# yzhang511/multi_modal_foundation_model

Hardware: NVIDIA B200
Metric: train trials/sec fwd+bwd (higher is better)
Workload: dtype bf16

## Files before the change

include/mmfm_b200.h:

```cpp
#ifndef MMFM_B200_H_
#define MMFM_B200_H_

#include <stddef.h>
#include <stdint.h>

#ifdef __cplusplus
extern "C" {
#endif

#define MMFM_ABI_VERSION 5

const char* mmfm_last_error(void);
int mmfm_abi_version(void);
int mmfm_sm_count(void);

typedef struct mmfm_dropout {
  const unsigned long long* seed;
  uint32_t site;
  uint32_t thresh;
  float scale;
} mmfm_dropout;

enum mmfm_act {
  MMFM_ACT_NONE = 0,
  MMFM_ACT_GELU = 1,
  MMFM_ACT_SOFTSIGN = 2,
  MMFM_ACT_DGELU = 3,
  MMFM_ACT_DSOFTSIGN = 4,
  MMFM_ACT_GELU_DG = 5,
  MMFM_ACT_MULAUX = 6,
  MMFM_ACT_ROWDOT_DROP = 7
};

typedef struct mmfm_gemm_args {
  const void* A; long long lda;
  const void* B; long long ldb;
  int M, N, K;
  void* D; long long ldd;
  int d_fp32;
  void* D2;
  const float* bias;
  const float* res; long long ldr;
  const void* aux; long long ldaux;
  int act; float act_scale;
  mmfm_dropout drop;
  int remap_T, remap_S, remap_off;
  const unsigned char* row_zero;
  float* rowdot; int rowdot_S;
} mmfm_gemm_args;

int mmfm_gemm_tn(const mmfm_gemm_args* args, void* stream);

int mmfm_gemm_wgrad(const void* dY, long long lddy, const void* X, long long ldx, int R, int NO, int KI, float* dW,
                    long long ldw, float* dbias, void* stream);
int mmfm_colsum_bf16(const void* dY, long long ld, int R, int NO, float* out, void* stream);

int mmfm_cast_bf16(const float* x, long long ldx, void* y, long long ldy, void* yt, long long ldyt, int R, int C,
                   void* stream);

int mmfm_layernorm_fwd(const float* x, const float* gamma, const float* beta, void* y, float* mean, float* rstd,
                       int R, int H, float eps, int modmajor_T, int S, void* stream);
int mmfm_layernorm_bwd(const void* dy, const float* x, const float* mean, const float* rstd, const float* gamma,
                       const float* dres, float* dx, void* dxb, const mmfm_dropout* drop, float* dgamma,
                       float* dbeta, int R, int H, int modmajor_T, int S, void* stream);

#define MMFM_MAX_LN 8
typedef struct {
  const float* x;
  int R, H, n;
  float eps;
  const float* gamma[MMFM_MAX_LN];
  const float* beta[MMFM_MAX_LN];
  void* y[MMFM_MAX_LN];
  float* mean;
  float* rstd;
  const void* dy[MMFM_MAX_LN];
  float* dgamma[MMFM_MAX_LN];
  float* dbeta[MMFM_MAX_LN];
  float* dx;
  void* dxb;
} mmfm_ln_multi_args;
int mmfm_layernorm_fwd_multi(const mmfm_ln_multi_args* a, void* stream);
int mmfm_layernorm_bwd_multi(const mmfm_ln_multi_args* a, void* stream);

int mmfm_scalenorm_fwd(const float* x, const float* g, void* y, float* rnorm, int R, int H, float eps, void* stream);
int mmfm_scalenorm_bwd(const void* dy, const float* x, const float* rnorm, const float* g, const float* dres, float* dx,
                       void* dxb, const mmfm_dropout* drop, float* dg, int R, int H, float eps, void* stream);

enum mmfm_mask_mode {
  MMFM_MASK_KEY = 0,
  MMFM_MASK_KEY_OR_DIAG = 1,
  MMFM_MASK_CAUSAL = 2
};
typedef struct mmfm_attn_args {
  const void* q; long long ldq;
  const void* k; long long ldk;
  const void* v; long long ldv;
  void* o; long long ldo;
  float* lse;
  const unsigned char* key_valid;
  const short* mod_q; const short* mod_k;
  int B, n_heads, Sq, Sk, d_head;
  int mask_mode;
  float scale;
  mmfm_dropout drop_p;
  mmfm_dropout drop_o;
  unsigned short* p_keep;
  void* d_o; long long lddo;
  float* delta;
  void* dq; long long lddq;
  void* dk; long long lddk;
  void* dv; long long lddv;
  int prep_done;
} mmfm_attn_args;
int mmfm_attention_fwd(const mmfm_attn_args* args, void* stream);
int mmfm_attention_bwd(const mmfm_attn_args* args, void* stream);

#define MMFM_MAX_MOD 8
typedef struct mmfm_mask_args {
  int n_mod, B, T;
  const long long* mask[MMFM_MAX_MOD]; long long mask_sb[MMFM_MAX_MOD]; long long mask_st[MMFM_MAX_MOD];
  const long long* attn[MMFM_MAX_MOD]; long long attn_sb[MMFM_MAX_MOD]; long long attn_st[MMFM_MAX_MOD];
  int channels[MMFM_MAX_MOD];
  const unsigned int* sample_thresh;
  const unsigned long long* seed;
} mmfm_mask_args;
#define MMFM_MASK_SITE 8192u
int mmfm_mask_prep(const mmfm_mask_args* args, unsigned char* zero_flags, unsigned char* key_valid,
                   unsigned char* tok_mask, long long* n_examples, float* inv_n, void* stream);
int mmfm_embed_assemble(const float* mod_emb_row, const float* pos_embed, const long long* ts, float* emb, int B,
                        int T, int S, int off, int H, void* stream);
int mmfm_embed_assemble_bwd(const float* g, const float* g2, const long long* ts, float* dpos, float* dmod, int B,
                            int T, int S, int off, int H, void* stream);
int mmfm_embed_grad_prep(const float* dx, void* dtok, const unsigned char* row_zero, const mmfm_dropout* drop, int B,
                         int T, int S, int off, int H, void* stream);
int mmfm_smallc_embed_fwd(const float* in, const float* W1, const float* b1, const float* W2, const float* b2,
                          const float* emb, float* x, float* hid, const unsigned char* row_zero,
                          const mmfm_dropout* drop, float act_scale, int act, int B, int T, int S, int off, int C,
                          int H, void* stream);
int mmfm_smallc_embed_bwd(const float* in, const float* hid, const float* W2, const float* dx,
                          const unsigned char* row_zero, const mmfm_dropout* drop, float act_scale, int act,
                          float* dW1, float* db1, float* dW2, float* db2, int B, int T, int S, int off, int C, int H,
                          void* stream);
int mmfm_smallc_head_fwd(const void* y, const float* W, const float* b, float* preds, int R, int H, int C,
                         void* stream);
int mmfm_smallc_head_bwd(const void* y, const float* W, const void* dpreds, long long lddp, void* dy, float* dW,
                         float* db, int R, int H, int C, void* stream);

enum mmfm_loss_kind {
  MMFM_LOSS_POISSON = 0, MMFM_LOSS_MSE = 1,
  MMFM_LOSS_CE = 2
};
int mmfm_loss_fwd_bwd(const float* preds, const float* targets, const unsigned char* tok_mask, int S, int off,
                      const float* inv_n, int kind, int B, int T, int C, float* partials, int n_partials, void* dpreds,
                      long long lddp, void* stream);
int mmfm_loss_finalize(const float* partials, int n_partials, int n_mod, const float* inv_n, float* mod_loss,
                       float* loss, void* stream);

typedef struct mmfm_cast_item {
  const float* src; long long ld_src;
  void* dst; long long ld_dst;
  void* dst_t; long long ld_dst_t;
  int rows, cols;
  int tile_start;
  int pad_;
} mmfm_cast_item;
int mmfm_cast_bf16_multi(const mmfm_cast_item* items_dev, int n_items, int total_tiles, void* stream);
int mmfm_scale_inplace(float* x, long long n, const float* scale_dev, void* stream);

int mmfm_csr_to_dense_u8(const unsigned char* data, const int* indices, const long long* row_ptr, long long n_rows, int N,
                         unsigned char* out, void* stream);
int mmfm_u8_expand(const unsigned char* x, long long R, int C, float* y32, long long ld32, void* y16, long long ld16,
                   void* stream);

int mmfm_column_stats(const float* pred, const float* y, long long R, int C, int log_rate, double* out, void* stream);

int mmfm_adamw_step(float* p, const float* g, float* exp_avg, float* exp_avg_sq, long long n, float lr, float beta1,
                    float beta2, float eps, float weight_decay, long long step, void* stream);

typedef struct mmfm_det_ws {
  void* buf;
  long long bytes;
  unsigned int* tickets;
  int n_tickets;
} mmfm_det_ws;
enum mmfm_det_kind {
  MMFM_DET_WGRAD = 0,
  MMFM_DET_COLSUM = 1,
  MMFM_DET_LN_BWD = 2,
  MMFM_DET_LN_BWD_MULTI = 3,
  MMFM_DET_SCALENORM_BWD = 4,
  MMFM_DET_EMBED_ASM_BWD = 5,
  MMFM_DET_SMALLC_EMBED_BWD = 6,
  MMFM_DET_SMALLC_HEAD_BWD = 7,
  MMFM_DET_COLUMN_STATS = 8
};
int mmfm_det_ws_bytes(int kind, long long d0, long long d1, long long d2, long long* bytes, int* n_tickets);
int mmfm_gemm_wgrad_det(const void* dY, long long lddy, const void* X, long long ldx, int R, int NO, int KI, float* dW,
                        long long ldw, float* dbias, const mmfm_det_ws* ws, void* stream);
int mmfm_colsum_bf16_det(const void* dY, long long ld, int R, int NO, float* out, const mmfm_det_ws* ws, void* stream);
int mmfm_layernorm_bwd_det(const void* dy, const float* x, const float* mean, const float* rstd, const float* gamma,
                           const float* dres, float* dx, void* dxb, const mmfm_dropout* drop, float* dgamma,
                           float* dbeta, int R, int H, int modmajor_T, int S, const mmfm_det_ws* ws, void* stream);
int mmfm_layernorm_bwd_multi_det(const mmfm_ln_multi_args* a, const mmfm_det_ws* ws, void* stream);
// ... 19 lines not shown
```

multi_modal_foundation_model_b200/_lib.py:

```python
from __future__ import annotations

import ctypes as C
import os
import subprocess
import sys
from typing import List, Optional

_PKG_DIR = os.path.dirname(os.path.abspath(__file__))
_CSRC = os.path.join(_PKG_DIR, "csrc")
LIB_PATH = os.environ.get("MMFM_LIB_PATH") or os.path.join(_PKG_DIR, "libmmfm_b200.so")
SOURCES = ["host_util.cu", "gemm.cu", "gemm_ts.cu", "norm.cu", "attention.cu", "attention_pipe.cu", "attention_bwd_stream.cu", "attention_bwd_persist.cu", "attention_bwd_ws.cu", "glue.cu"]
NVCC_FLAGS = ["-gencode", "arch=compute_100a,code=sm_100a", "-lineinfo", "-O3", "-std=c++17", "-Xcompiler", "-fPIC",
              "-Xptxas", "-v"]

MAX_MOD = 8
ABI_VERSION = 5
MASK_SITE = 8192


def _nvcc() -> str:
    for p in (os.environ.get("NVCC"), "/usr/local/cuda/bin/nvcc", "nvcc"):
        if p and (os.path.isabs(p) and os.path.exists(p) or not os.path.isabs(p)):
            return p
    return "nvcc"


def needs_build() -> bool:
    if not os.path.exists(LIB_PATH):
        return True
    t = os.path.getmtime(LIB_PATH)
    deps = [os.path.join(_CSRC, f) for f in os.listdir(_CSRC)]
    deps.append(os.path.join(os.path.dirname(_PKG_DIR), "include", "mmfm_b200.h"))
    return any(os.path.getmtime(d) > t for d in deps if os.path.exists(d))


def build(force: bool = False, verbose: bool = False) -> str:
    if not force and not needs_build():
        return LIB_PATH
    objs: List[str] = []
    build_dir = os.path.join(_PKG_DIR, "build")
    os.makedirs(build_dir, exist_ok=True)
    procs = []
    for src in SOURCES:
        obj = os.path.join(build_dir, src.replace(".cu", ".o"))
        objs.append(obj)
        extra = os.environ.get("MMFM_NVCC_EXTRA", "").split()
        cmd = [_nvcc(), *NVCC_FLAGS, *extra, "-c", os.path.join(_CSRC, src), "-o", obj]
        procs.append((src, subprocess.Popen(cmd, stdout=subprocess.PIPE, stderr=subprocess.STDOUT, text=True)))
    for src, p in procs:
        out, _ = p.communicate()
        if verbose or p.returncode != 0:
            sys.stderr.write(out)
        if p.returncode != 0:
            raise RuntimeError(f"nvcc failed on {src}")
    cmd = [_nvcc(), "-shared", "-o", LIB_PATH, *objs, "-lcudart"]
    r = subprocess.run(cmd, stdout=subprocess.PIPE, stderr=subprocess.STDOUT, text=True)
    if r.returncode != 0:
        sys.stderr.write(r.stdout)
        raise RuntimeError("link of libmmfm_b200.so failed")
    return LIB_PATH


class Dropout(C.Structure):
    _fields_ = [("seed", C.c_void_p), ("site", C.c_uint32), ("thresh", C.c_uint32), ("scale", C.c_float)]


class GemmArgs(C.Structure):
    _fields_ = [
        ("A", C.c_void_p), ("lda", C.c_longlong),
        ("B", C.c_void_p), ("ldb", C.c_longlong),
        ("M", C.c_int), ("N", C.c_int), ("K", C.c_int),
        ("D", C.c_void_p), ("ldd", C.c_longlong),
        ("d_fp32", C.c_int),
        ("D2", C.c_void_p),
        ("bias", C.c_void_p),
        ("res", C.c_void_p), ("ldr", C.c_longlong),
        ("aux", C.c_void_p), ("ldaux", C.c_longlong),
        ("act", C.c_int), ("act_scale", C.c_float),
        ("drop", Dropout),
        ("remap_T", C.c_int), ("remap_S", C.c_int), ("remap_off", C.c_int),
        ("row_zero", C.c_void_p),
        ("rowdot", C.c_void_p), ("rowdot_S", C.c_int),
    ]


class AttnArgs(C.Structure):
    _fields_ = [
        ("q", C.c_void_p), ("ldq", C.c_longlong),
        ("k", C.c_void_p), ("ldk", C.c_longlong),
        ("v", C.c_void_p), ("ldv", C.c_longlong),
        ("o", C.c_void_p), ("ldo", C.c_longlong),
        ("lse", C.c_void_p),
        ("key_valid", C.c_void_p),
        ("mod_q", C.c_void_p), ("mod_k", C.c_void_p),
        ("B", C.c_int), ("n_heads", C.c_int), ("Sq", C.c_int), ("Sk", C.c_int), ("d_head", C.c_int),
        ("mask_mode", C.c_int),
        ("scale", C.c_float),
        ("drop_p", Dropout), ("drop_o", Dropout),
        ("p_keep", C.c_void_p),
        ("d_o", C.c_void_p), ("lddo", C.c_longlong),
        ("delta", C.c_void_p),
        ("dq", C.c_void_p), ("lddq", C.c_longlong),
        ("dk", C.c_void_p), ("lddk", C.c_longlong),
        ("dv", C.c_void_p), ("lddv", C.c_longlong),
        ("prep_done", C.c_int),
    ]


class MaskArgs(C.Structure):
    _fields_ = [
        ("n_mod", C.c_int), ("B", C.c_int), ("T", C.c_int),
        ("mask", C.c_void_p * MAX_MOD), ("mask_sb", C.c_longlong * MAX_MOD), ("mask_st", C.c_longlong * MAX_MOD),
        ("attn", C.c_void_p * MAX_MOD), ("attn_sb", C.c_longlong * MAX_MOD), ("attn_st", C.c_longlong * MAX_MOD),
        ("channels", C.c_int * MAX_MOD),
        ("sample_thresh", C.c_void_p), ("seed", C.c_void_p),
    ]


MAX_LN = 8


class LnMultiArgs(C.Structure):
    _fields_ = [
        ("x", C.c_void_p), ("R", C.c_int), ("H", C.c_int), ("n", C.c_int), ("eps", C.c_float),
        ("gamma", C.c_void_p * MAX_LN), ("beta", C.c_void_p * MAX_LN), ("y", C.c_void_p * MAX_LN),
        ("mean", C.c_void_p), ("rstd", C.c_void_p),
        ("dy", C.c_void_p * MAX_LN), ("dgamma", C.c_void_p * MAX_LN), ("dbeta", C.c_void_p * MAX_LN),
        ("dx", C.c_void_p), ("dxb", C.c_void_p),
    ]


class CastItem(C.Structure):
    _fields_ = [
        ("src", C.c_void_p), ("ld_src", C.c_longlong),
        ("dst", C.c_void_p), ("ld_dst", C.c_longlong),
        ("dst_t", C.c_void_p), ("ld_dst_t", C.c_longlong),
        ("rows", C.c_int), ("cols", C.c_int),
        ("tile_start", C.c_int), ("pad_", C.c_int),
    ]


class DetWs(C.Structure):
    _fields_ = [("buf", C.c_void_p), ("bytes", C.c_longlong), ("tickets", C.c_void_p), ("n_tickets", C.c_int)]


ACT_NONE, ACT_GELU, ACT_SOFTSIGN, ACT_DGELU, ACT_DSOFTSIGN, ACT_GELU_DG, ACT_MULAUX, ACT_ROWDOT_DROP = 0, 1, 2, 3, 4, 5, 6, 7
MASK_KEY, MASK_KEY_OR_DIAG, MASK_CAUSAL = 0, 1, 2
LOSS_POISSON, LOSS_MSE, LOSS_CE = 0, 1, 2
(DET_WGRAD, DET_COLSUM, DET_LN_BWD, DET_LN_BWD_MULTI, DET_SCALENORM_BWD, DET_EMBED_ASM_BWD, DET_SMALLC_EMBED_BWD,
 DET_SMALLC_HEAD_BWD, DET_COLUMN_STATS) = range(9)

_vp, _i, _ll, _f = C.c_void_p, C.c_int, C.c_longlong, C.c_float
_DP = C.POINTER(Dropout)
_WS = C.POINTER(DetWs)

SIGNATURES = {
    "mmfm_gemm_tn": [C.POINTER(GemmArgs), _vp],
    "mmfm_gemm_wgrad": [_vp, _ll, _vp, _ll, _i, _i, _i, _vp, _ll, _vp, _vp],
    "mmfm_colsum_bf16": [_vp, _ll, _i, _i, _vp, _vp],
    "mmfm_cast_bf16": [_vp, _ll, _vp, _ll, _vp, _ll, _i, _i, _vp],
    "mmfm_cast_bf16_multi": [_vp, _i, _i, _vp],
    "mmfm_scale_inplace": [_vp, _ll, _vp, _vp],
    "mmfm_csr_to_dense_u8": [_vp, _vp, _vp, _ll, _i, _vp, _vp],
    "mmfm_u8_expand": [_vp, _ll, _i, _vp, _ll, _vp, _ll, _vp],
    "mmfm_column_stats": [_vp, _vp, _ll, _i, _i, _vp, _vp],
    "mmfm_adamw_step": [_vp, _vp, _vp, _vp, _ll, _f, _f, _f, _f, _f, _ll, _vp],
    "mmfm_layernorm_fwd": [_vp, _vp, _vp, _vp, _vp, _vp, _i, _i, _f, _i, _i, _vp],
    "mmfm_layernorm_bwd": [_vp, _vp, _vp, _vp, _vp, _vp, _vp, _vp, _DP, _vp, _vp, _i, _i, _i, _i, _vp],
    "mmfm_layernorm_fwd_multi": [C.POINTER(LnMultiArgs), _vp],
    "mmfm_layernorm_bwd_multi": [C.POINTER(LnMultiArgs), _vp],
    "mmfm_scalenorm_fwd": [_vp, _vp, _vp, _vp, _i, _i, _f, _vp],
    "mmfm_scalenorm_bwd": [_vp, _vp, _vp, _vp, _vp, _vp, _vp, _DP, _vp, _i, _i, _f, _vp],
    "mmfm_attention_fwd": [C.POINTER(AttnArgs), _vp],
    "mmfm_attention_bwd": [C.POINTER(AttnArgs), _vp],
    "mmfm_mask_prep": [C.POINTER(MaskArgs), _vp, _vp, _vp, _vp, _vp, _vp],
    "mmfm_embed_assemble": [_vp, _vp, _vp, _vp, _i, _i, _i, _i, _i, _vp],
    "mmfm_embed_assemble_bwd": [_vp, _vp, _vp, _vp, _vp, _i, _i, _i, _i, _i, _vp],
    "mmfm_embed_grad_prep": [_vp, _vp, _vp, _DP, _i, _i, _i, _i, _i, _vp],
    "mmfm_smallc_embed_fwd": [_vp, _vp, _vp, _vp, _vp, _vp, _vp, _vp, _vp, _DP, _f, _i, _i, _i, _i, _i, _i, _i, _vp],
    "mmfm_smallc_embed_bwd": [_vp, _vp, _vp, _vp, _vp, _DP, _f, _i, _vp, _vp, _vp, _vp, _i, _i, _i, _i, _i, _i, _vp],
    "mmfm_smallc_head_fwd": [_vp, _vp, _vp, _vp, _i, _i, _i, _vp],
    "mmfm_smallc_head_bwd": [_vp, _vp, _vp, _ll, _vp, _vp, _vp, _i, _i, _i, _vp],
    "mmfm_loss_fwd_bwd": [_vp, _vp, _vp, _i, _i, _vp, _i, _i, _i, _i, _vp, _i, _vp, _ll, _vp],
    "mmfm_loss_finalize": [_vp, _i, _i, _vp, _vp, _vp, _vp],
    "mmfm_det_ws_bytes": [_i, _ll, _ll, _ll, C.POINTER(C.c_longlong), C.POINTER(C.c_int)],
    "mmfm_gemm_wgrad_det": [_vp, _ll, _vp, _ll, _i, _i, _i, _vp, _ll, _vp, _WS, _vp],
    "mmfm_colsum_bf16_det": [_vp, _ll, _i, _i, _vp, _WS, _vp],
    "mmfm_layernorm_bwd_det": [_vp, _vp, _vp, _vp, _vp, _vp, _vp, _vp, _DP, _vp, _vp, _i, _i, _i, _i, _WS, _vp],
    "mmfm_layernorm_bwd_multi_det": [C.POINTER(LnMultiArgs), _WS, _vp],
    "mmfm_scalenorm_bwd_det": [_vp, _vp, _vp, _vp, _vp, _vp, _vp, _DP, _vp, _i, _i, _f, _WS, _vp],
    "mmfm_embed_assemble_bwd_det": [_vp, _vp, _vp, _vp, _vp, _i, _i, _i, _i, _i, _i, _WS, _vp],
    "mmfm_smallc_embed_bwd_det": [_vp, _vp, _vp, _vp, _vp, _DP, _f, _i, _vp, _vp, _vp, _vp, _i, _i, _i, _i, _i, _i, _WS,
                                  _vp],
    "mmfm_smallc_head_bwd_det": [_vp, _vp, _vp, _ll, _vp, _vp, _vp, _i, _i, _i, _WS, _vp],
    "mmfm_column_stats_det": [_vp, _vp, _ll, _i, _i, _vp, _WS, _vp],
}
_SPECIAL = {
    "mmfm_last_error": ([], C.c_char_p),
    "mmfm_abi_version": ([], C.c_int),
    "mmfm_sm_count": ([], C.c_int),
}
EXPORTED_SYMBOLS = sorted(list(SIGNATURES) + list(_SPECIAL))

_LIB: Optional[C.CDLL] = None


class MmfmError(RuntimeError):
    pass


def lib() -> C.CDLL:
    global _LIB
    if _LIB is not None:
        return _LIB
    if not os.path.exists(LIB_PATH):
        raise MmfmError(
            f"{LIB_PATH} is missing: build it with `python -c 'import __graft_entry__ as g; g.build()'` "
            "(nvcc, sm_100a).  The B200 path has no CPU / PyTorch fallback.")
    L = C.CDLL(LIB_PATH)
    for name, argtypes in SIGNATURES.items():
        fn = getattr(L, name)
        fn.argtypes = argtypes
        fn.restype = C.c_int
    for name, (argtypes, restype) in _SPECIAL.items():
        fn = getattr(L, name)
        fn.argtypes = argtypes
        fn.restype = restype
    if L.mmfm_abi_version() != ABI_VERSION:
        raise MmfmError("libmmfm_b200.so ABI version mismatch")
    _LIB = L
    return L


def check(rc: int, what: str = "") -> None:
    if rc != 0:
        msg = lib().mmfm_last_error()
        raise MmfmError(f"{what} failed (rc={rc}): {msg.decode() if msg else '?'}")
```

multi_modal_foundation_model_b200/csrc/common.cuh:

```cuda
#pragma once
#include <cuda.h>
#include <cuda_bf16.h>
#include <cuda_runtime.h>
#include <stdint.h>
#include <stdio.h>

namespace mmfm {

typedef __nv_bfloat16 bf16;

#define MMFM_DEVINL __device__ __forceinline__

MMFM_DEVINL uint32_t smem_u32(const void* p) { return (uint32_t)__cvta_generic_to_shared(p); }

MMFM_DEVINL bool elect_one() {
  uint32_t pred = 0;
  asm volatile(
      "{\n\t.reg .pred P1;\n\t.reg .b32 R1;\n\t"
      "elect.sync R1|P1, 0xffffffff;\n\t"
      "selp.u32 %0, 1, 0, P1;\n\t}\n"
      : "=r"(pred));
  return pred != 0;
}

// ... 161 lines not shown
}

MMFM_DEVINL void tmem_ld32(uint32_t taddr, uint32_t (&r)[32]) {
  asm volatile(
      "tcgen05.ld.sync.aligned.32x32b.x32.b32 "
      "{%0, %1, %2, %3, %4, %5, %6, %7, %8, %9, %10, %11, %12, %13, %14, %15, "
      "%16, %17, %18, %19, %20, %21, %22, %23, %24, %25, %26, %27, %28, %29, %30, %31}, [%32];"
      : "=r"(r[0]), "=r"(r[1]), "=r"(r[2]), "=r"(r[3]), "=r"(r[4]), "=r"(r[5]), "=r"(r[6]), "=r"(r[7]),
        "=r"(r[8]), "=r"(r[9]), "=r"(r[10]), "=r"(r[11]), "=r"(r[12]), "=r"(r[13]), "=r"(r[14]), "=r"(r[15]),
        "=r"(r[16]), "=r"(r[17]), "=r"(r[18]), "=r"(r[19]), "=r"(r[20]), "=r"(r[21]), "=r"(r[22]),
        "=r"(r[23]), "=r"(r[24]), "=r"(r[25]), "=r"(r[26]), "=r"(r[27]), "=r"(r[28]), "=r"(r[29]),
        "=r"(r[30]), "=r"(r[31])
      : "r"(taddr)
      : "memory");
}
MMFM_DEVINL void tmem_ld16(uint32_t taddr, uint32_t (&r)[16]) {
  asm volatile(
      "tcgen05.ld.sync.aligned.32x32b.x16.b32 "
      "{%0, %1, %2, %3, %4, %5, %6, %7, %8, %9, %10, %11, %12, %13, %14, %15}, [%16];"
      : "=r"(r[0]), "=r"(r[1]), "=r"(r[2]), "=r"(r[3]), "=r"(r[4]), "=r"(r[5]), "=r"(r[6]), "=r"(r[7]),
        "=r"(r[8]), "=r"(r[9]), "=r"(r[10]), "=r"(r[11]), "=r"(r[12]), "=r"(r[13]), "=r"(r[14]), "=r"(r[15])
      : "r"(taddr)
      : "memory");
}
MMFM_DEVINL void tmem_ld_wait() { asm volatile("tcgen05.wait::ld.sync.aligned;" ::: "memory"); }
MMFM_DEVINL void tmem_st16(uint32_t taddr, const uint32_t (&r)[16]) {
  asm volatile(
      "tcgen05.st.sync.aligned.32x32b.x16.b32 [%0], "
      "{%1, %2, %3, %4, %5, %6, %7, %8, %9, %10, %11, %12, %13, %14, %15, %16};" ::"r"(taddr),
      "r"(r[0]), "r"(r[1]), "r"(r[2]), "r"(r[3]), "r"(r[4]), "r"(r[5]), "r"(r[6]), "r"(r[7]), "r"(r[8]), "r"(r[9]),
      "r"(r[10]), "r"(r[11]), "r"(r[12]), "r"(r[13]), "r"(r[14]), "r"(r[15])
      : "memory");
}
MMFM_DEVINL void tmem_st8(uint32_t taddr, const uint32_t (&r)[8]) {
  asm volatile("tcgen05.st.sync.aligned.32x32b.x8.b32 [%0], {%1, %2, %3, %4, %5, %6, %7, %8};" ::"r"(taddr), "r"(r[0]),
               "r"(r[1]), "r"(r[2]), "r"(r[3]), "r"(r[4]), "r"(r[5]), "r"(r[6]), "r"(r[7])
               : "memory");
}
MMFM_DEVINL void tmem_st_wait() { asm volatile("tcgen05.wait::st.sync.aligned;" ::: "memory"); }

MMFM_DEVINL uint64_t make_smem_desc(uint32_t saddr, uint32_t lbo_bytes, uint32_t sbo_bytes, uint32_t layout) {
  uint64_t d = 0;
  d |= (uint64_t)((saddr >> 4) & 0x3FFF);
  d |= (uint64_t)((lbo_bytes >> 4) & 0x3FFF) << 16;
  d |= (uint64_t)((sbo_bytes >> 4) & 0x3FFF) << 32;
  d |= (uint64_t)1 << 46;
  d |= (uint64_t)(layout & 7) << 61;
  return d;
}
__host__ __device__ inline uint32_t make_idesc_bf16(uint32_t M, uint32_t N, uint32_t a_mn, uint32_t b_mn) {
  uint32_t d = 0;
  d |= 1u << 4;
  d |= 1u << 7;
  d |= 1u << 10;
  d |= (a_mn & 1u) << 15;
  d |= (b_mn & 1u) << 16;
  d |= ((N >> 3) & 0x3F) << 17;
  d |= ((M >> 4) & 0x1F) << 24;
  return d;
}

constexpr int kPhiloxRounds = 7;

MMFM_DEVINL void mulhilo32(uint32_t a, uint32_t b, uint32_t& hi, uint32_t& lo) {
  const unsigned long long p = (unsigned long long)a * (unsigned long long)b;
  hi = (uint32_t)(p >> 32);
  lo = (uint32_t)p;
}

MMFM_DEVINL uint4 philox4x32(uint32_t c0, uint32_t c1, uint32_t c2, uint32_t c3, uint32_t k0, uint32_t k1) {
#pragma unroll
  for (int r = 0; r < kPhiloxRounds; ++r) {
    uint32_t hi0, lo0, hi1, lo1;
    mulhilo32(0xD2511F53u, c0, hi0, lo0);
    mulhilo32(0xCD9E8D57u, c2, hi1, lo1);
    const uint32_t n0 = hi1 ^ c1 ^ k0;
    const uint32_t n2 = hi0 ^ c3 ^ k1;
    c0 = n0; c1 = lo1; c2 = n2; c3 = lo0;
    k0 += 0x9E3779B9u; k1 += 0xBB67AE85u;
  }
  return make_uint4(c0, c1, c2, c3);
}

MMFM_DEVINL void philox4x32_x4(uint32_t c0, uint32_t c1, uint32_t c2, uint32_t c3, uint32_t k0, uint32_t k1,
                               uint4 (&out)[4]) {
  uint32_t a0[4], a1[4], a2[4], a3[4];
#pragma unroll
  for (int q = 0; q < 4; ++q) { a0[q] = c0 + q; a1[q] = c1; a2[q] = c2; a3[q] = c3; }
#pragma unroll
  for (int r = 0; r < kPhiloxRounds; ++r) {
#pragma unroll
    for (int q = 0; q < 4; ++q) {
      uint32_t hi0, lo0, hi1, lo1;
      mulhilo32(0xD2511F53u, a0[q], hi0, lo0);
      mulhilo32(0xCD9E8D57u, a2[q], hi1, lo1);
      const uint32_t n0 = hi1 ^ a1[q] ^ k0;
      const uint32_t n2 = hi0 ^ a3[q] ^ k1;
      a0[q] = n0; a1[q] = lo1; a2[q] = n2; a3[q] = lo0;
    }
    k0 += 0x9E3779B9u; k1 += 0xBB67AE85u;
  }
#pragma unroll
  for (int q = 0; q < 4; ++q) out[q] = make_uint4(a0[q], a1[q], a2[q], a3[q]);
}

struct DropCfg {
  const unsigned long long* seed;
  uint32_t site;
  uint32_t thresh;
  float scale;
};

MMFM_DEVINL uint4 drop_bytes16(unsigned long long seed, uint32_t site, uint64_t row, uint32_t groups_per_row,
                               uint32_t g16) {
  uint64_t g = row * (uint64_t)groups_per_row + g16;
  return philox4x32((uint32_t)g, (uint32_t)(g >> 32), site, 0u, (uint32_t)seed, (uint32_t)(seed >> 32));
}
MMFM_DEVINL uint32_t drop_byte(const uint4& w, int b) {
  uint32_t word = (b < 4) ? w.x : (b < 8) ? w.y : (b < 12) ? w.z : w.w;
  return (word >> ((b & 3) * 8)) & 0xFFu;
}

MMFM_DEVINL float erf_poly(float z, float& e) {
  const float az = fabsf(z);
  float t, ex;
  asm("rcp.approx.ftz.f32 %0, %1;" : "=f"(t) : "f"(fmaf(0.3275911f, az, 1.0f)));
  asm("ex2.approx.ftz.f32 %0, %1;" : "=f"(ex) : "f"(-1.4426950408889634f * z * z));
  e = ex;
  const float poly =
      fmaf(fmaf(fmaf(fmaf(1.061405429f, t, -1.453152027f), t, 1.421413741f), t, -0.284496736f), t, 0.254829592f) * t;
  return copysignf(fmaf(-poly, ex, 1.0f), z);
}
MMFM_DEVINL float gelu_erf(float x) {
  float e;
  return 0.5f * x * (1.0f + erf_poly(x * 0.70710678118654752f, e));
}
MMFM_DEVINL float gelu_erf_grad(float x) {
  float e;
  const float cdf = 0.5f * (1.0f + erf_poly(x * 0.70710678118654752f, e));
  return fmaf(x * 0.3989422804014327f, e, cdf);
}
MMFM_DEVINL void gelu_erf_both(float x, float& g, float& dg) {
  float e;
  const float cdf = 0.5f * (1.0f + erf_poly(x * 0.70710678118654752f, e));
  g = x * cdf;
  dg = fmaf(x * 0.3989422804014327f, e, cdf);
}
MMFM_DEVINL float softsign(float x) { return x / (1.0f + fabsf(x)); }

MMFM_DEVINL float warp_sum(float v) {
#pragma unroll
  for (int o = 16; o > 0; o >>= 1) v += __shfl_xor_sync(0xffffffffu, v, o);
  return v;
}

MMFM_DEVINL uint32_t pack_bf16x2(float lo, float hi) {
  __nv_bfloat162 v = __floats2bfloat162_rn(lo, hi);
  return *reinterpret_cast<uint32_t*>(&v);
}
MMFM_DEVINL float2 unpack_bf16x2(uint32_t u) {
  __nv_bfloat162 v = *reinterpret_cast<__nv_bfloat162*>(&u);
  return __bfloat1622float2(v);
}


MMFM_DEVINL uint64_t pack_f2(float lo, float hi) {
  uint64_t r;
  asm("mov.b64 %0, {%1, %2};" : "=l"(r) : "f"(lo), "f"(hi));
  return r;
}
MMFM_DEVINL void unpack_f2(uint64_t v, float& lo, float& hi) { asm("mov.b64 {%0, %1}, %2;" : "=f"(lo), "=f"(hi) : "l"(v)); }
MMFM_DEVINL uint64_t ffma2(uint64_t a, uint64_t b, uint64_t c) {
  uint64_t d;
  asm("fma.rn.f32x2 %0, %1, %2, %3;" : "=l"(d) : "l"(a), "l"(b), "l"(c));
  return d;
}
MMFM_DEVINL uint64_t fmul2(uint64_t a, uint64_t b) {
  uint64_t d;
  asm("mul.rn.f32x2 %0, %1, %2;" : "=l"(d) : "l"(a), "l"(b));
  return d;
}
MMFM_DEVINL uint64_t fadd2(uint64_t a, uint64_t b) {
  uint64_t d;
  asm("add.rn.f32x2 %0, %1, %2;" : "=l"(d) : "l"(a), "l"(b));
  return d;
}

MMFM_DEVINL void gelu_erf_both2(float x0, float x1, float& g0, float& g1, float& d0, float& d1) {
  const uint64_t x = pack_f2(x0, x1);
  const uint64_t z = fmul2(x, pack_f2(0.70710678118654752f, 0.70710678118654752f));
  float z0, z1;
  unpack_f2(z, z0, z1);
  float t0, t1, e0, e1;
  asm("rcp.approx.ftz.f32 %0, %1;" : "=f"(t0) : "f"(fmaf(0.3275911f, fabsf(z0), 1.0f)));
  asm("rcp.approx.ftz.f32 %0, %1;" : "=f"(t1) : "f"(fmaf(0.3275911f, fabsf(z1), 1.0f)));
  float a0, a1;
  unpack_f2(fmul2(fmul2(z, z), pack_f2(-1.4426950408889634f, -1.4426950408889634f)), a0, a1);
  asm("ex2.approx.ftz.f32 %0, %1;" : "=f"(e0) : "f"(a0));
  asm("ex2.approx.ftz.f32 %0, %1;" : "=f"(e1) : "f"(a1));
  const uint64_t t = pack_f2(t0, t1), e = pack_f2(e0, e1);
  uint64_t q = ffma2(pack_f2(1.061405429f, 1.061405429f), t, pack_f2(-1.453152027f, -1.453152027f));
  q = ffma2(q, t, pack_f2(1.421413741f, 1.421413741f));
  q = ffma2(q, t, pack_f2(-0.284496736f, -0.284496736f));
  q = ffma2(q, t, pack_f2(0.254829592f, 0.254829592f));
  q = fmul2(q, t);
  float r0, r1;
  unpack_f2(ffma2(q, fmul2(e, pack_f2(-1.0f, -1.0f)), pack_f2(1.0f, 1.0f)), r0, r1);
  const uint64_t erf2 = pack_f2(copysignf(r0, z0), copysignf(r1, z1));
  const uint64_t cdf = ffma2(erf2, pack_f2(0.5f, 0.5f), pack_f2(0.5f, 0.5f));
  unpack_f2(fmul2(x, cdf), g0, g1);
  unpack_f2(ffma2(fmul2(x, pack_f2(0.3989422804014327f, 0.3989422804014327f)), e, cdf), d0, d1);
}

MMFM_DEVINL void ldsm_x4(uint32_t (&r)[4], uint32_t saddr) {
  asm volatile("ldmatrix.sync.aligned.m8n8.x4.shared.b16 {%0,%1,%2,%3}, [%4];"
               : "=r"(r[0]), "=r"(r[1]), "=r"(r[2]), "=r"(r[3])
               : "r"(saddr));
}
MMFM_DEVINL void ldsm_x4_t(uint32_t (&r)[4], uint32_t saddr) {
  asm volatile("ldmatrix.sync.aligned.m8n8.x4.trans.shared.b16 {%0,%1,%2,%3}, [%4];"
               : "=r"(r[0]), "=r"(r[1]), "=r"(r[2]), "=r"(r[3])
               : "r"(saddr));
}
MMFM_DEVINL void mma_16816(float (&d)[4], const uint32_t (&a)[4], const uint32_t (&b)[2]) {
  asm volatile(
      "mma.sync.aligned.m16n8k16.row.col.f32.bf16.bf16.f32 {%0,%1,%2,%3}, {%4,%5,%6,%7}, {%8,%9}, {%0,%1,%2,%3};"
      : "+f"(d[0]), "+f"(d[1]), "+f"(d[2]), "+f"(d[3])
      : "r"(a[0]), "r"(a[1]), "r"(a[2]), "r"(a[3]), "r"(b[0]), "r"(b[1]));
}

MMFM_DEVINL void mma_16816_z(float (&d)[4], const uint32_t (&a)[4], const uint32_t (&b)[2]) {
  asm volatile(
      "mma.sync.aligned.m16n8k16.row.col.f32.bf16.bf16.f32 {%0,%1,%2,%3}, {%4,%5,%6,%7}, {%8,%9}, {%10,%10,%10,%10};"
      : "=f"(d[0]), "=f"(d[1]), "=f"(d[2]), "=f"(d[3])
      : "r"(a[0]), "r"(a[1]), "r"(a[2]), "r"(a[3]), "r"(b[0]), "r"(b[1]), "f"(0.f));
}

MMFM_DEVINL float quad_sum(float v) {
  v += __shfl_xor_sync(0xffffffffu, v, 1);
  v += __shfl_xor_sync(0xffffffffu, v, 2);
  return v;
}
MMFM_DEVINL float quad_max(float v) {
  v = fmaxf(v, __shfl_xor_sync(0xffffffffu, v, 1));
  v = fmaxf(v, __shfl_xor_sync(0xffffffffu, v, 2));
  return v;
}

MMFM_DEVINL float det_add(float a, float b) { return a + b; }
MMFM_DEVINL double det_add(double a, double b) { return a + b; }
MMFM_DEVINL float4 det_add(float4 a, float4 b) { return make_float4(a.x + b.x, a.y + b.y, a.z + b.z, a.w + b.w); }

template <typename V, typename Emit>
MMFM_DEVINL void det_tree_fold(V* ws, long long stride, int n, int leaf, int n_leaves, unsigned int* tickets,
                               Emit emit) {
  __shared__ unsigned int s_second;
  int node = leaf;
  for (int l = 0; (1 << l) < n_leaves; ++l) {
    const int width = (n_leaves + (1 << l) - 1) >> l;
    if ((node | 1) >= width) { node >>= 1; continue; }
    const int right = (node | 1) << l;
    __syncthreads();
    if (threadIdx.x == 0) {
      __threadfence();
      const unsigned int t = atomicAdd(tickets + right - 1, 1u);
      if (t != 0u) {
        tickets[right - 1] = 0u;
        __threadfence();
      }
      s_second = t;
    }
    __syncthreads();
    if (s_second == 0u) return;
    V* a = ws + (long long)((node & ~1) << l) * stride;
    const V* b = ws + (long long)right * stride;
    constexpr int kU = 8;
    for (int i0 = threadIdx.x; i0 < n; i0 += kU * blockDim.x) {
      V va[kU], vb[kU];
#pragma unroll
      for (int u = 0; u < kU; ++u) {
        const int i = i0 + u * blockDim.x;
        if (i < n) { va[u] = __ldcg(a + i); vb[u] = __ldcg(b + i); }
      }
#pragma unroll
      for (int u = 0; u < kU; ++u) {
        const int i = i0 + u * blockDim.x;
        if (i >= n) break;
        if (width == 2) emit(i, det_add(va[u], vb[u]));
        else a[i] = det_add(va[u], vb[u]);
      }
    }
    if (width == 2) return;
    node >>= 1;
  }
  __syncthreads();
  for (int i = threadIdx.x; i < n; i += blockDim.x) emit(i, __ldcg(ws + (long long)leaf * stride + i));
}

MMFM_DEVINL uint32_t drop_byte_at(unsigned long long seed, uint32_t site, uint64_t row, uint32_t groups_per_row,
                                  uint32_t col) {
  uint4 w = drop_bytes16(seed, site, row, groups_per_row, col >> 4);
  return drop_byte(w, col & 15);
}

}
```

multi_modal_foundation_model_b200/csrc/gemm.cu:

```cuda
#include "common.cuh"
#include <stdlib.h>
#include "host_util.h"
#include "../../include/mmfm_b200.h"

namespace mmfm {

constexpr int kBM = 128;
constexpr int kBK = 64;
constexpr int kGemmThreads = 192;

MMFM_DEVINL float4 ld4_f32(const float* p, bool vec, int nvalid) {
  if (vec) return __ldg(reinterpret_cast<const float4*>(p));
  float4 r = make_float4(0.f, 0.f, 0.f, 0.f);
  if (nvalid > 0) r.x = __ldg(p);
  if (nvalid > 1) r.y = __ldg(p + 1);
  if (nvalid > 2) r.z = __ldg(p + 2);
  if (nvalid > 3) r.w = __ldg(p + 3);
  return r;
}
MMFM_DEVINL float4 ld4_bf16(const bf16* p, bool vec, int nvalid) {
  if (vec) {
    const uint2 u = __ldg(reinterpret_cast<const uint2*>(p));
    const float2 a = unpack_bf16x2(u.x), b = unpack_bf16x2(u.y);
    return make_float4(a.x, a.y, b.x, b.y);
  }
  float4 r = make_float4(0.f, 0.f, 0.f, 0.f);
  if (nvalid > 0) r.x = __bfloat162float(p[0]);
  if (nvalid > 1) r.y = __bfloat162float(p[1]);
  if (nvalid > 2) r.z = __bfloat162float(p[2]);
  if (nvalid > 3) r.w = __bfloat162float(p[3]);
  return r;
}
MMFM_DEVINL void st4_f32(float* p, bool vec, int nvalid, const float4& v) {
  if (vec) { *reinterpret_cast<float4*>(p) = v; return; }
  if (nvalid > 0) p[0] = v.x;
  if (nvalid > 1) p[1] = v.y;
  if (nvalid > 2) p[2] = v.z;
  if (nvalid > 3) p[3] = v.w;
}
MMFM_DEVINL void st4_bf16(bf16* p, bool vec, int nvalid, const float4& v) {
  if (vec) { *reinterpret_cast<uint2*>(p) = make_uint2(pack_bf16x2(v.x, v.y), pack_bf16x2(v.z, v.w)); return; }
  if (nvalid > 0) p[0] = __float2bfloat16_rn(v.x);
  if (nvalid > 1) p[1] = __float2bfloat16_rn(v.y);
  if (nvalid > 2) p[2] = __float2bfloat16_rn(v.z);
  if (nvalid > 3) p[3] = __float2bfloat16_rn(v.w);
}

constexpr int kEpiWarps = 16;
constexpr int kTnThreads = 64 + kEpiWarps * 32;

enum EpiKind : int {
  EPI_PLAIN_BF16 = 0,
  EPI_PLAIN_F32 = 1,
  EPI_RES_F32 = 2,
  EPI_GELU = 3,
  EPI_SOFTSIGN = 4,
  EPI_DGELU = 5,
  EPI_DSOFTSIGN = 6,
  EPI_GENERIC = 7,
  EPI_GELU_DG = 8,
  EPI_MULAUX = 9
};

template <int BN, int STAGES, int EPI>
__global__ void __launch_bounds__(kTnThreads, 1) gemm_tn_kernel(const __grid_constant__ CUtensorMap tmA,
                                                                 const __grid_constant__ CUtensorMap tmB,
                                                                 const mmfm_gemm_args p, int tiles_n, int n_tiles,
                                                                 int bstat) {
  constexpr uint32_t kABytes = kBM * kBK * 2;
  constexpr uint32_t kBBytes = BN * kBK * 2;
  constexpr uint32_t kStageBytes = kABytes + kBBytes;
  constexpr uint32_t kTmemCols = 2 * BN;
  constexpr int kPitch = BN + 4;
  constexpr int kHalf = BN / (kEpiWarps / 4);
  constexpr bool GEN = EPI == EPI_GENERIC;

  constexpr int kMaxStages = 8;
  extern __shared__ uint8_t smem_raw[];
  __shared__ __align__(8) uint64_t full_bar[kMaxStages];
  __shared__ __align__(8) uint64_t empty_bar[kMaxStages];
  __shared__ __align__(8) uint64_t b_full;
  __shared__ __align__(8) uint64_t acc_full[2];
  __shared__ __align__(8) uint64_t acc_empty[2];
  __shared__ uint32_t tmem_slot;
  __shared__ __align__(16) float s_bias[kEpiWarps][kHalf];

  const uint32_t smem_base = (smem_u32(smem_raw) + 1023u) & ~1023u;
  float* stage_f = reinterpret_cast<float*>(smem_raw + (smem_base - smem_u32(smem_raw)) + STAGES * kStageBytes);
  const int warp = threadIdx.x >> 5;
  const int lane = threadIdx.x & 31;
  const int nkb = (p.K + kBK - 1) / kBK;
  const uint32_t b_res_bytes = bstat ? (uint32_t)nkb * kBBytes : 0u;
  const uint32_t ring_base = smem_base + b_res_bytes;
  const uint32_t st_bytes = bstat ? kABytes : kStageBytes;
  uint32_t nst = bstat ? (STAGES * kStageBytes - b_res_bytes) / kABytes : (uint32_t)STAGES;
  if (nst > (uint32_t)kMaxStages) nst = kMaxStages;

  pdl_trigger();
  if (warp == 0 && lane == 0) {
    tma_prefetch_desc(&tmA);
    tma_prefetch_desc(&tmB);
#pragma unroll
    for (int s = 0; s < kMaxStages; ++s) {
      mbar_init(&full_bar[s], 1);
      mbar_init(&empty_bar[s], 1);
    }
    mbar_init(&b_full, 1);
    mbar_init(&acc_full[0], 1);
    mbar_init(&acc_full[1], 1);
    mbar_init(&acc_empty[0], kEpiWarps);
    mbar_init(&acc_empty[1], kEpiWarps);
    fence_mbar_init();
  }
  if (warp == 1) {
    tmem_alloc(&tmem_slot, kTmemCols);
    tmem_relinquish();
  }
  tc_fence_before();
  __syncthreads();
  tc_fence_after();
  const uint32_t tmem_base = tmem_slot;
  pdl_wait();

  if (warp == 0) {
    if (elect_one()) {
      uint32_t it = 0;
      if (bstat) {
        const int n0 = ((int)blockIdx.x % tiles_n) * BN;
        mbar_arrive_expect_tx(&b_full, b_res_bytes);
        for (int kb = 0; kb < nkb; ++kb) tma_load_2d_addr(smem_base + kb * kBBytes, &tmB, &b_full, kb * kBK, n0);
      }
      for (int tile = blockIdx.x; tile < n_tiles; tile += gridDim.x) {
        const int m0 = (tile / tiles_n) * kBM, n0 = (tile % tiles_n) * BN;
        {
          const int t2 = tile + 2 * (int)gridDim.x;
          if (t2 < n_tiles && (t2 % tiles_n == 0 || tiles_n > (int)gridDim.x)) {
            const int m2 = (t2 / tiles_n) * kBM;
            for (int kb = 0; kb < nkb; ++kb) tma_prefetch_l2_2d(&tmA, kb * kBK, m2);
          }
        }
        for (int kb = 0; kb < nkb; ++kb, ++it) {
          const uint32_t s = it % nst;
          if (it >= nst) mbar_wait(&empty_bar[s], ((it / nst) - 1) & 1);
          mbar_arrive_expect_tx(&full_bar[s], st_bytes);
          const uint32_t a_dst = ring_base + s * st_bytes;
          tma_load_2d_addr(a_dst, &tmA, &full_bar[s], kb * kBK, m0);
          if (!bstat) tma_load_2d_addr(a_dst + kABytes, &tmB, &full_bar[s], kb * kBK, n0);
        }
      }
    }
  } else if (warp == 1) {
    if (elect_one()) {
      const uint32_t idesc = make_idesc_bf16(kBM, BN, 0, 0);
      uint32_t it = 0, t = 0;
      if (bstat) mbar_wait(&b_full, 0);
      for (int tile = blockIdx.x; tile < n_tiles; tile += gridDim.x, ++t) {
        const uint32_t buf = t & 1u;
        if (t >= 2) mbar_wait(&acc_empty[buf], ((t >> 1) - 1) & 1);
        tc_fence_after();
        const uint32_t d_tmem = tmem_base + buf * BN;
        for (int kb = 0; kb < nkb; ++kb, ++it) {
          const uint32_t s = it % nst;
          mbar_wait(&full_bar[s], (it / nst) & 1);
          tc_fence_after();
          const uint32_t a_addr = ring_base + s * st_bytes;
          const uint32_t b_addr = bstat ? smem_base + kb * kBBytes : a_addr + kABytes;
#pragma unroll
          for (int k = 0; k < kBK / 16; ++k) {
            const uint64_t da = make_smem_desc(a_addr + k * 32, 16, 1024, 2);
            const uint64_t db = make_smem_desc(b_addr + k * 32, 16, 1024, 2);
            umma_bf16(d_tmem, da, db, idesc, (kb > 0 || k > 0) ? 1u : 0u);
          }
          umma_commit(&empty_bar[s]);
        }
        umma_commit(&acc_full[buf]);
      }
    }
  } else {
    const int ew = warp - 2;
    const int quad = warp & 3;
    const int half = ew >> 2;
    const int cbase = half * kHalf;
    const int row_l = quad * 32 + lane;
    constexpr bool kMayDrop = GEN || EPI == EPI_RES_F32;
    constexpr bool kHasRes = GEN || EPI == EPI_RES_F32;
    constexpr bool kHasAux = GEN || EPI == EPI_DGELU || EPI == EPI_DSOFTSIGN || EPI == EPI_MULAUX;
    bool drop = false;
    unsigned long long seed = 0ull;
    if (kMayDrop) {
      drop = p.drop.thresh != 0u;
      if (drop) seed = *p.drop.seed;
    }
    const uint32_t drop_gpr = (uint32_t)((p.N + 15) >> 4);
    const int act = GEN ? p.act : 0;
    const bool f32out = GEN ? (p.d_fp32 != 0) : (EPI == EPI_PLAIN_F32 || EPI == EPI_RES_F32);
    const float inv_scale = 1.0f / p.act_scale;
    const bool has_res = GEN ? (p.res != nullptr) : (EPI == EPI_RES_F32);
    const bool has_aux = GEN ? (act == MMFM_ACT_DGELU || act == MMFM_ACT_DSOFTSIGN || act == MMFM_ACT_MULAUX) : kHasAux;
    float* my_bias = s_bias[ew];
    static_assert(kHalf <= 64, "bias slice: at most two values per lane");
    auto load_bias = [&](int tile_i, float (&b)[2]) {
      b[0] = b[1] = 0.f;
      if (tile_i < n_tiles && p.bias) {
        const int nn = (tile_i % tiles_n) * BN + cbase;
        if (lane < kHalf && nn + lane < p.N) b[0] = __ldg(p.bias + nn + lane);
        if (lane + 32 < kHalf && nn + lane + 32 < p.N) b[1] = __ldg(p.bias + nn + lane + 32);
      }
    };
    float bias_next[2];
    load_bias(blockIdx.x, bias_next);

    uint32_t t = 0;
    for (int tile = blockIdx.x; tile < n_tiles; tile += gridDim.x, ++t) {
      const uint32_t buf = t & 1u;
      const int m0 = (tile / tiles_n) * kBM, n0 = (tile % tiles_n) * BN;
      const long long r = (long long)m0 + row_l;
      const bool warp_has_cols = (n0 + cbase) < p.N;
      if (lane < kHalf) my_bias[lane] = bias_next[0];
      if (lane + 32 < kHalf) my_bias[lane + 32] = bias_next[1];
      load_bias(tile + gridDim.x, bias_next);
      bool zero = false;
      if (kMayDrop && p.row_zero && r < p.M) {
        const int pos = p.remap_T > 0 ? p.remap_off + (int)(r % p.remap_T) : (int)(r % p.remap_S);
        zero = p.row_zero[pos] != 0;
      }
      if (r < p.M && warp_has_cols) {
        const int ncols = min(kHalf, p.N - n0 - cbase);
        if (kHasRes && p.res) {
          long long orow = r;
          if (p.remap_T > 0) {
            const int bb = (int)r / p.remap_T;
            orow = (long long)bb * p.remap_S + p.remap_off + ((int)r - bb * p.remap_T);
          }
          const char* ptr = reinterpret_cast<const char*>(p.res + orow * p.ldr + n0 + cbase);
          for (int o = 0; o < ncols * 4; o += 128) asm volatile("prefetch.global.L2 [%0];" ::"l"(ptr + o));
        }
        if (kHasAux && p.aux) {
          const char* ptr =
              reinterpret_cast<const char*>(reinterpret_cast<const bf16*>(p.aux) + r * p.ldaux + n0 + cbase);
          for (int o = 0; o < ncols * 2; o += 128) asm volatile("prefetch.global.L2 [%0];" ::"l"(ptr + o));
        }
      }
      __syncwarp();
      mbar_wait(&acc_full[buf], (t >> 1) & 1);
      tc_fence_after();
      const bool interior = (m0 + kBM <= p.M) && (n0 + BN <= p.N);
      if ((EPI == EPI_PLAIN_BF16 || EPI == EPI_RES_F32) && interior && p.remap_T == 0 && kHalf == 32) {
        const uint32_t t_row = tmem_base + buf * BN + ((uint32_t)(quad * 32) << 16) + (uint32_t)cbase;
        if (EPI == EPI_PLAIN_BF16) {
          constexpr int kPitchH = BN + 8;
          bf16* stage_h = reinterpret_cast<bf16*>(stage_f);
          bf16* my_row_h = stage_h + row_l * kPitchH + cbase;
#pragma unroll
          for (int c0 = 0; c0 < 32; c0 += 16) {
            uint32_t acc[16];
            tmem_ld16(t_row + (uint32_t)c0, acc);
            tmem_ld_wait();
            uint32_t h[8];
#pragma unroll
            for (int j4 = 0; j4 < 4; ++j4) {
              const float4 b4 = *reinterpret_cast<const float4*>(&my_bias[c0 + j4 * 4]);
              h[2 * j4] = pack_bf16x2(__uint_as_float(acc[4 * j4]) + b4.x, __uint_as_float(acc[4 * j4 + 1]) + b4.y);
              h[2 * j4 + 1] = pack_bf16x2(__uint_as_float(acc[4 * j4 + 2]) + b4.z, __uint_as_float(acc[4 * j4 + 3]) + b4.w);
            }
            *reinterpret_cast<uint4*>(my_row_h + c0) = make_uint4(h[0], h[1], h[2], h[3]);
            *reinterpret_cast<uint4*>(my_row_h + c0 + 8) = make_uint4(h[4], h[5], h[6], h[7]);
          }
          tc_fence_before();
          __syncwarp();
          if (lane == 0) mbar_arrive(&acc_empty[buf]);
          const int lr = (lane >> 3) + 4 * ((lane >> 2) & 1), lc = (lane & 3) * 8;
          bf16* dst = reinterpret_cast<bf16*>(p.D) + ((long long)m0 + quad * 32 + lr) * p.ldd + n0 + cbase + lc;
          const bf16* src = stage_h + (quad * 32 + lr) * kPitchH + cbase + lc;
#pragma unroll
          for (int st8 = 0; st8 < 4; ++st8)
            *reinterpret_cast<uint4*>(dst + (long long)st8 * 8 * p.ldd) = *reinterpret_cast<const uint4*>(src + st8 * 8 * kPitchH);
        } else {
          float* my_row = stage_f + row_l * kPitch + cbase;
#pragma unroll
          for (int c0 = 0; c0 < 32; c0 += 16) {
            uint32_t acc[16];
            tmem_ld16(t_row + (uint32_t)c0, acc);
            tmem_ld_wait();
            float v[16];
#pragma unroll
            for (int j4 = 0; j4 < 4; ++j4) {
              const float4 b4 = *reinterpret_cast<const float4*>(&my_bias[c0 + j4 * 4]);
              v[4 * j4 + 0] = __uint_as_float(acc[4 * j4 + 0]) + b4.x;
              v[4 * j4 + 1] = __uint_as_float(acc[4 * j4 + 1]) + b4.y;
              v[4 * j4 + 2] = __uint_as_float(acc[4 * j4 + 2]) + b4.z;
              v[4 * j4 + 3] = __uint_as_float(acc[4 * j4 + 3]) + b4.w;
            }
            if (drop) {
              const uint4 w = drop_bytes16(seed, p.drop.site, (uint64_t)r, drop_gpr, (uint32_t)((n0 + cbase + c0) >> 4));
#pragma unroll
              for (int j = 0; j < 16; ++j) v[j] = (drop_byte(w, j) < p.drop.thresh) ? 0.f : v[j] * p.drop.scale;
            }
            if (zero) {
#pragma unroll
              for (int j = 0; j < 16; ++j) v[j] = 0.f;
            }
#pragma unroll
            for (int j4 = 0; j4 < 4; ++j4)
              *reinterpret_cast<float4*>(my_row + c0 + j4 * 4) =
                  make_float4(v[4 * j4], v[4 * j4 + 1], v[4 * j4 + 2], v[4 * j4 + 3]);
          }
          tc_fence_before();
          __syncwarp();
          if (lane == 0) mbar_arrive(&acc_empty[buf]);
          const int lr = lane >> 3, lc = (lane & 7) * 4;
          const long long grow = (long long)m0 + quad * 32 + lr;
          const float* rsrc = p.res + grow * p.ldr + n0 + cbase + lc;
          float* dst = reinterpret_cast<float*>(p.D) + grow * p.ldd + n0 + cbase + lc;
          const float* src = stage_f + (quad * 32 + lr) * kPitch + cbase + lc;
          float4 rv[8];
#pragma unroll
          for (int s8 = 0; s8 < 8; ++s8) rv[s8] = __ldg(reinterpret_cast<const float4*>(rsrc + (long long)s8 * 4 * p.ldr));
#pragma unroll
          for (int s8 = 0; s8 < 8; ++s8) {
            const float4 v = *reinterpret_cast<const float4*>(src + s8 * 4 * kPitch);
            *reinterpret_cast<float4*>(dst + (long long)s8 * 4 * p.ldd) =
                make_float4(v.x + rv[s8].x, v.y + rv[s8].y, v.z + rv[s8].z, v.w + rv[s8].w);
          }
        }
        __syncwarp();
        continue;
      }
      if (warp_has_cols) {
        const uint32_t t_row = tmem_base + buf * BN + ((uint32_t)(quad * 32) << 16) + (uint32_t)cbase;
        float* my_row = stage_f + row_l * kPitch + cbase;
#pragma unroll
        for (int c0 = 0; c0 < kHalf; c0 += 16) {
          uint32_t acc[16];
          tmem_ld16(t_row + (uint32_t)c0, acc);
          tmem_ld_wait();
          float v[16];
#pragma unroll
          for (int j4 = 0; j4 < 4; ++j4) {
            const float4 b4 = *reinterpret_cast<const float4*>(&my_bias[c0 + j4 * 4]);
            v[4 * j4 + 0] = __uint_as_float(acc[4 * j4 + 0]) + b4.x;
            v[4 * j4 + 1] = __uint_as_float(acc[4 * j4 + 1]) + b4.y;
            v[4 * j4 + 2] = __uint_as_float(acc[4 * j4 + 2]) + b4.z;
            v[4 * j4 + 3] = __uint_as_float(acc[4 * j4 + 3]) + b4.w;
          }
          if (kMayDrop) {
            if (drop) {
              const uint4 w = drop_bytes16(seed, p.drop.site, (uint64_t)r, drop_gpr, (uint32_t)((n0 + cbase + c0) >> 4));
#pragma unroll
              for (int j = 0; j < 16; ++j) v[j] = (drop_byte(w, j) < p.drop.thresh) ? 0.f : v[j] * p.drop.scale;
            }
            if (zero) {
#pragma unroll
              for (int j = 0; j < 16; ++j) v[j] = 0.f;
            }
          }
#pragma unroll
          for (int j4 = 0; j4 < 4; ++j4)
            *reinterpret_cast<float4*>(my_row + c0 + j4 * 4) =
                make_float4(v[4 * j4], v[4 * j4 + 1], v[4 * j4 + 2], v[4 * j4 + 3]);
        }
      }
      tc_fence_before();
      __syncwarp();
      if (lane == 0) mbar_arrive(&acc_empty[buf]);
      if (warp_has_cols) {
        constexpr int kLanesPerRow = kHalf / 4;
        constexpr int kRowsPerStep = 32 / kLanesPerRow;
        constexpr int kSteps = 32 / kRowsPerStep;
        constexpr int kBatch = kSteps < 8 ? kSteps : 8;
// ... 213 lines not shown
      tmem_ld32(t_row + (uint32_t)c0, acc);
      tmem_ld_wait();
#pragma unroll
      for (int j4 = 0; j4 < 8; ++j4)
        *reinterpret_cast<float4*>(my_row + c0 + j4 * 4) =
            make_float4(__uint_as_float(acc[4 * j4]), __uint_as_float(acc[4 * j4 + 1]),
                        __uint_as_float(acc[4 * j4 + 2]), __uint_as_float(acc[4 * j4 + 3]));
    }
    if (do_bias) {
      uint32_t bacc[16];
      tmem_ld16(t_row + (uint32_t)BN, bacc);
      tmem_ld_wait();
      if constexpr (DET) {
        float* slot = reinterpret_cast<float*>(ws + (blockIdx.z + (long long)gridDim.z * (blockIdx.y * gridDim.x + blockIdx.x)) *
                                                        wgrad_slot_f4<BN>());
        slot[kBM * BN + row_l] = __uint_as_float(bacc[0]);
      } else {
        if (no0 + row_l < NO) atomicAdd(dbias + no0 + row_l, __uint_as_float(bacc[0]));
      }
    }
    __syncwarp();
#pragma unroll 1
    for (int cp = 0; cp < BN / 128; ++cp) {
      const int lcol = cp * 128 + lane * 4;
      const int kcol = ki0 + lcol;
      const int nvalid = KI - kcol;
      const bool vec = (ldw % 4 == 0) && nvalid >= 4 && ((reinterpret_cast<uintptr_t>(dW) & 15) == 0);
#pragma unroll 4
      for (int it = 0; it < 32; ++it) {
        const int rl = quad * 32 + it;
        const int no = no0 + rl;
        if (no >= NO || nvalid <= 0) continue;
        const float4 v = *reinterpret_cast<const float4*>(stage_f + rl * kPitch + lcol);
        if constexpr (DET) {
          ws[(blockIdx.z + (long long)gridDim.z * (blockIdx.y * gridDim.x + blockIdx.x)) * wgrad_slot_f4<BN>() +
             (rl * BN + lcol) / 4] = v;
          continue;
        }
        float* dst = dW + (long long)no * ldw + kcol;
        if (vec) {
          asm volatile("red.global.add.v4.f32 [%0], {%1, %2, %3, %4};" ::"l"(dst), "f"(v.x), "f"(v.y), "f"(v.z),
                       "f"(v.w)
                       : "memory");
        } else {
          if (nvalid > 0) atomicAdd(dst, v.x);
          if (nvalid > 1) atomicAdd(dst + 1, v.y);
          if (nvalid > 2) atomicAdd(dst + 2, v.z);
          if (nvalid > 3) atomicAdd(dst + 3, v.w);
        }
      }
    }
  }
  tc_fence_before();
  __syncthreads();
  if (clustered) cluster_sync_all();
  if (warp == 1) tmem_dealloc(tmem_base, kTmemCols);
  if constexpr (DET) {
    const long long tile = blockIdx.y * gridDim.x + blockIdx.x;
    const bool vec = (ldw % 4 == 0) && ((reinterpret_cast<uintptr_t>(dW) & 15) == 0);
    det_tree_fold(ws + tile * gridDim.z * wgrad_slot_f4<BN>(), wgrad_slot_f4<BN>(),
                  (kBM * BN + (do_bias ? kBM : 0)) / 4, blockIdx.z, gridDim.z, tickets + tile * gridDim.z,
                  [&](int i, float4 v) {
                    const int e = 4 * i;
                    if (e >= kBM * BN) {
                      const float vv[4] = {v.x, v.y, v.z, v.w};
                      for (int u = 0; u < 4; ++u)
                        if (no0 + e - kBM * BN + u < NO) dbias[no0 + e - kBM * BN + u] += vv[u];
                      return;
                    }
                    const int no = no0 + e / BN, kcol = ki0 + e % BN;
                    if (no >= NO || kcol >= KI) return;
                    float* dst = dW + (long long)no * ldw + kcol;
                    if (vec && kcol + 4 <= KI) {
                      float4 o = *reinterpret_cast<float4*>(dst);
                      *reinterpret_cast<float4*>(dst) = det_add(o, v);
                      return;
                    }
                    const float vv[4] = {v.x, v.y, v.z, v.w};
                    for (int u = 0; u < 4 && kcol + u < KI; ++u) dst[u] += vv[u];
                  });
  }
}

constexpr int kColsumRows = 256;
template <bool DET = false>
__global__ void __launch_bounds__(256) colsum_bf16_kernel(const bf16* __restrict__ dY, long long ld, int R, int NO,
                                                           float* __restrict__ out, float* __restrict__ ws,
                                                           unsigned int* tickets) {
  const int c = (blockIdx.x * 256 + threadIdx.x) * 2;
  if (!DET && c >= NO) return;
  const int r0 = blockIdx.y * kColsumRows;
  const int r1 = (DET && c >= NO) ? r0 : min(R, r0 + kColsumRows);
  float s0 = 0.f, s1 = 0.f;
  if (c + 1 < NO && (ld & 1) == 0) {
    for (int r = r0; r < r1; ++r) {
      uint32_t u = __ldg(reinterpret_cast<const uint32_t*>(dY + (long long)r * ld + c));
      float2 f = unpack_bf16x2(u);
      s0 += f.x;
      s1 += f.y;
    }
  } else {
    for (int r = r0; r < r1; ++r) {
      s0 += __bfloat162float(dY[(long long)r * ld + c]);
      if (c + 1 < NO) s1 += __bfloat162float(dY[(long long)r * ld + c + 1]);
    }
  }
  if constexpr (DET) {
    float* slices = ws + (long long)blockIdx.x * gridDim.y * 512;
    slices[blockIdx.y * 512 + 2 * threadIdx.x] = s0;
    slices[blockIdx.y * 512 + 2 * threadIdx.x + 1] = s1;
    det_tree_fold(slices, 512, 512, blockIdx.y, gridDim.y, tickets + (long long)blockIdx.x * gridDim.y,
                  [&](int i, float v) {
                    if (blockIdx.x * 512 + i < NO) out[blockIdx.x * 512 + i] += v;
                  });
    return;
  }
  atomicAdd(out + c, s0);
  if (c + 1 < NO) atomicAdd(out + c + 1, s1);
}

__global__ void __launch_bounds__(256) cast_bf16_kernel(const float* __restrict__ x, long long ldx, bf16* __restrict__ y,
                                                         long long ldy, bf16* __restrict__ yt, long long ldyt, int R,
                                                         int C) {
  __shared__ float tile[32][33];
  const int c0 = blockIdx.x * 32, r0 = blockIdx.y * 32;
  const int tx = threadIdx.x & 31, ty = threadIdx.x >> 5;
#pragma unroll
  for (int i = 0; i < 4; ++i) {
    const int r = r0 + ty + i * 8, c = c0 + tx;
    float v = 0.f;
    if (r < R && c < C) {
      v = x[(long long)r * ldx + c];
      if (y) y[(long long)r * ldy + c] = __float2bfloat16_rn(v);
    }
    tile[ty + i * 8][tx] = v;
  }
  if (yt == nullptr) return;
  __syncthreads();
#pragma unroll
  for (int i = 0; i < 4; ++i) {
    const int c = c0 + ty + i * 8, r = r0 + tx;
    if (r < R && c < C) yt[(long long)c * ldyt + r] = __float2bfloat16_rn(tile[tx][ty + i * 8]);
  }
}

}

namespace mmfm {
int try_launch_gemm_ts(const mmfm_gemm_args* a, cudaStream_t st);
}
using namespace mmfm;

template <int BN, int STAGES, int EPI>
static int launch_tn(const mmfm_gemm_args* a, cudaStream_t st) {
  CUtensorMap tmA, tmB;
  int rc = make_tmap_bf16_2d(&tmA, a->A, (uint64_t)a->M, (uint64_t)a->K, (uint64_t)a->lda, kBK, kBM, TMA_SW_128);
  if (rc) return rc;
  rc = make_tmap_bf16_2d(&tmB, a->B, (uint64_t)a->N, (uint64_t)a->K, (uint64_t)a->ldb, kBK, BN, TMA_SW_128);
  if (rc) return rc;
  constexpr size_t smem = (size_t)STAGES * (kBM * kBK * 2 + BN * kBK * 2) + (size_t)kBM * (BN + 4) * 4 + 1024;
  static bool attr_set = false;
  if (!attr_set) {
    MMFM_CHECK_CUDA(cudaFuncSetAttribute(gemm_tn_kernel<BN, STAGES, EPI>, cudaFuncAttributeMaxDynamicSharedMemorySize,
                                         (int)smem));
    attr_set = true;
  }
  const int tiles_n = (a->N + BN - 1) / BN, tiles_m = (a->M + kBM - 1) / kBM;
  const int n_tiles = tiles_n * tiles_m;
  int grid = n_tiles < device_sm_count() ? n_tiles : device_sm_count();
  static int bstat_env = -1;
  if (bstat_env < 0) {
    const char* e = getenv("MMFM_GEMM_BSTAT");
    bstat_env = (e && e[0] == '1') ? 1 : 0;
  }
  const int nkb = (a->K + kBK - 1) / kBK;
  int bstat = 0;
  if (bstat_env && (size_t)nkb * BN * kBK * 2 * 2 <= (size_t)STAGES * (kBM * kBK * 2 + BN * kBK * 2) &&
      tiles_n <= device_sm_count() && tiles_m > 1) {
    int per_n = device_sm_count() / tiles_n;
    if (per_n > tiles_m) per_n = tiles_m;
    grid = per_n * tiles_n;
    bstat = 1;
  }
  set_l2_window(a->D, (size_t)a->M * (size_t)a->ldd * (a->d_fp32 ? 4 : 2));
  MMFM_CHECK_CUDA(launch_pdl(gemm_tn_kernel<BN, STAGES, EPI>, dim3(grid), dim3(kTnThreads), smem, st, tmA, tmB, *a, tiles_n,
                             n_tiles, bstat));
  return 0;
}

template <int EPI>
static int launch_tn_bn(const mmfm_gemm_args* a, cudaStream_t st) {
  if (a->N <= 64) return launch_tn<64, 4, EPI>(a, st);
  return launch_tn<128, 4, EPI>(a, st);
}

static bool al(const void* p, uintptr_t m) { return (reinterpret_cast<uintptr_t>(p) & (m - 1)) == 0; }

static int pick_epi(const mmfm_gemm_args* a) {
  if (a->N % 4 != 0 || a->ldd % 4 != 0) return EPI_GENERIC;
  const bool f32 = a->d_fp32 != 0;
  if (!al(a->D, f32 ? 16 : 8)) return EPI_GENERIC;
  const bool extras = a->drop.thresh != 0 || a->row_zero != nullptr || a->remap_T > 0;
  if (a->res) {
    if (a->act != MMFM_ACT_NONE || !f32 || a->D2 || a->ldr % 4 != 0 || !al(a->res, 16)) return EPI_GENERIC;
    return EPI_RES_F32;
  }
  if (extras) return EPI_GENERIC;
  switch (a->act) {
    case MMFM_ACT_NONE: return a->D2 ? EPI_GENERIC : (f32 ? EPI_PLAIN_F32 : EPI_PLAIN_BF16);
    case MMFM_ACT_GELU: return (!f32 && a->D2 && al(a->D2, 8)) ? EPI_GELU : EPI_GENERIC;
    case MMFM_ACT_GELU_DG: return (!f32 && a->D2 && al(a->D2, 8)) ? EPI_GELU_DG : EPI_GENERIC;
    case MMFM_ACT_MULAUX:
      if (f32 || a->D2 || a->ldaux % 4 != 0 || !al(a->aux, 8)) return EPI_GENERIC;
      return EPI_MULAUX;
    case MMFM_ACT_SOFTSIGN: return (!f32 && !a->D2) ? EPI_SOFTSIGN : EPI_GENERIC;
    case MMFM_ACT_DGELU:
    case MMFM_ACT_DSOFTSIGN:
      if (f32 || a->D2 || a->ldaux % 4 != 0 || !al(a->aux, 8)) return EPI_GENERIC;
      return a->act == MMFM_ACT_DGELU ? EPI_DGELU : EPI_DSOFTSIGN;
  }
  return EPI_GENERIC;
}

extern "C" int mmfm_gemm_tn(const mmfm_gemm_args* a, void* stream) {
  MMFM_REQUIRE(a != nullptr, "mmfm_gemm_tn: null args");
  MMFM_REQUIRE(a->M > 0 && a->N > 0 && a->K > 0, "mmfm_gemm_tn: bad shape M=%d N=%d K=%d", a->M, a->N, a->K);
  MMFM_REQUIRE(a->A && a->B && a->D, "mmfm_gemm_tn: null operand");
  MMFM_REQUIRE(a->act >= MMFM_ACT_NONE && a->act <= MMFM_ACT_ROWDOT_DROP, "mmfm_gemm_tn: bad act %d", a->act);
  MMFM_REQUIRE(!(a->act == MMFM_ACT_DGELU || a->act == MMFM_ACT_DSOFTSIGN || a->act == MMFM_ACT_MULAUX ||
                 a->act == MMFM_ACT_ROWDOT_DROP) || a->aux,
               "mmfm_gemm_tn: act %d needs aux", a->act);
  MMFM_REQUIRE(a->act != MMFM_ACT_ROWDOT_DROP || (a->rowdot && a->rowdot_S > 0 && a->M % a->rowdot_S == 0),
               "mmfm_gemm_tn: MMFM_ACT_ROWDOT_DROP needs rowdot / rowdot_S with M %% rowdot_S == 0");
  MMFM_REQUIRE(a->act != MMFM_ACT_GELU_DG || a->D2, "mmfm_gemm_tn: MMFM_ACT_GELU_DG needs the D2 buffer");
  MMFM_REQUIRE(a->drop.thresh == 0 || a->drop.seed, "mmfm_gemm_tn: dropout without seed pointer");
  MMFM_REQUIRE(a->drop.thresh < 256, "mmfm_gemm_tn: dropout threshold out of range");
  MMFM_REQUIRE(!(a->row_zero && a->remap_T == 0) || a->remap_S > 0, "mmfm_gemm_tn: row_zero needs remap_S");
  MMFM_REQUIRE(a->act == MMFM_ACT_NONE || a->act == MMFM_ACT_ROWDOT_DROP || (a->drop.thresh == 0 && a->row_zero == nullptr),
               "mmfm_gemm_tn: an activation epilogue cannot be combined with dropout / token zeroing");
  cudaStream_t st = (cudaStream_t)stream;
  {
    const int taken = try_launch_gemm_ts(a, st);
    if (taken != 0) return taken > 0 ? 0 : taken;
    MMFM_REQUIRE(a->act != MMFM_ACT_ROWDOT_DROP,
                 "mmfm_gemm_tn: MMFM_ACT_ROWDOT_DROP is built for the TMA-store kernel only (bf16 D, N %% 32 == 0, N > 64, "
                 "16-byte aligned D / aux / pitches, no remap / bias)");
  }
  switch (pick_epi(a)) {
    case EPI_PLAIN_BF16: return launch_tn_bn<EPI_PLAIN_BF16>(a, st);
    case EPI_PLAIN_F32: return launch_tn_bn<EPI_PLAIN_F32>(a, st);
    case EPI_RES_F32: return launch_tn_bn<EPI_RES_F32>(a, st);
    case EPI_GELU: return launch_tn_bn<EPI_GELU>(a, st);
    case EPI_SOFTSIGN: return launch_tn_bn<EPI_SOFTSIGN>(a, st);
    case EPI_DGELU: return launch_tn_bn<EPI_DGELU>(a, st);
    case EPI_DSOFTSIGN: return launch_tn_bn<EPI_DSOFTSIGN>(a, st);
    case EPI_GELU_DG: return launch_tn_bn<EPI_GELU_DG>(a, st);
    case EPI_MULAUX: return launch_tn_bn<EPI_MULAUX>(a, st);
    default: return launch_tn_bn<EPI_GENERIC>(a, st);
  }
}

static int wgrad_splits(int R, int NO, int KI, int BN, int* rows_per_split) {
  const int tiles = ((NO + kBM - 1) / kBM) * ((KI + BN - 1) / BN);
  const int kblocks = (R + kBK - 1) / kBK;
  static int waves_x2 = -1;
  if (waves_x2 < 0) {
    const char* e = getenv("MMFM_WGRAD_CTAS_X2");
    waves_x2 = e ? atoi(e) : 4;
    if (waves_x2 < 1) waves_x2 = 4;
  }
  int splits = ((BN == 256 ? 2 : waves_x2) * device_sm_count() / 2) / tiles;
  if (splits > kblocks) splits = kblocks;
  if (splits < 1) splits = 1;
  *rows_per_split = ((kblocks + splits - 1) / splits) * kBK;
  return (R + *rows_per_split - 1) / *rows_per_split;
}

template <int BN>
static int launch_wgrad(const void* dY, long long lddy, const void* X, long long ldx, int R, int NO, int KI, float* dW,
                        long long ldw, float* dbias, void* stream) {
  constexpr int STAGES = 3;
  CUtensorMap tmY, tmX;
  int rc = make_tmap_bf16_2d(&tmY, dY, (uint64_t)R, (uint64_t)NO, (uint64_t)lddy, 64, kBK, TMA_SW_128);
  if (rc) return rc;
  rc = make_tmap_bf16_2d(&tmX, X, (uint64_t)R, (uint64_t)KI, (uint64_t)ldx, 64, kBK, TMA_SW_128);
  if (rc) return rc;
  constexpr size_t smem = (size_t)STAGES * ((2 + BN / 64) * 64 * kBK * 2) + 2048 + 1024;
  static bool attr_set = false;
  if (!attr_set) {
    MMFM_CHECK_CUDA(cudaFuncSetAttribute(gemm_wgrad_kernel<STAGES, BN>, cudaFuncAttributeMaxDynamicSharedMemorySize,
                                         (int)smem));
    attr_set = true;
  }
  int rows_per_split = 0;
  const int splits = wgrad_splits(R, NO, KI, BN, &rows_per_split);
  dim3 grid((KI + BN - 1) / BN, (NO + kBM - 1) / kBM, splits);
  static int mc_env = -1;
  if (mc_env < 0) {
    const char* e = getenv("MMFM_WGRAD_MULTICAST");
    mc_env = (e && e[0] == '1') ? 1 : 0;
  }
  const int cx = (mc_env && BN == 128 && grid.x % 2 == 0) ? 2 : 1, cy = (mc_env && BN == 128 && grid.y % 2 == 0) ? 2 : 1;
  cudaLaunchConfig_t cfg = {};
  cfg.gridDim = grid;
  cfg.blockDim = dim3(kGemmThreads);
  cfg.dynamicSmemBytes = smem;
  cfg.stream = (cudaStream_t)stream;
  cudaLaunchAttribute attr[2];
  attr[0].id = cudaLaunchAttributeClusterDimension;
  attr[0].val.clusterDim.x = cx;
  attr[0].val.clusterDim.y = cy;
  attr[0].val.clusterDim.z = 1;
  attr[1].id = cudaLaunchAttributeProgrammaticStreamSerialization;
  attr[1].val.programmaticStreamSerializationAllowed = pdl_enabled() ? 1 : 0;
  cfg.attrs = attr;
  cfg.numAttrs = 2;
  MMFM_CHECK_CUDA(cudaLaunchKernelEx(&cfg, gemm_wgrad_kernel<STAGES, BN>, tmY, tmX, R, NO, KI, dW, ldw, rows_per_split, dbias,
                                     cx, cy, (float4*)nullptr, (unsigned int*)nullptr));
  return 0;
}

static DetNeed wgrad_det_need(int R, int NO, int KI) {
  int rows_per_split = 0;
  const int splits = wgrad_splits(R, NO, KI, 128, &rows_per_split);
  const long long ctas = (long long)((NO + kBM - 1) / kBM) * ((KI + 127) / 128) * splits;
  return DetNeed{ctas * wgrad_slot_f4<128>() * 16, (int)ctas};
}

static int launch_wgrad_det(const void* dY, long long lddy, const void* X, long long ldx, int R, int NO, int KI,
                            float* dW, long long ldw, float* dbias, const mmfm_det_ws* ws, cudaStream_t st) {
  constexpr int STAGES = 3, BN = 128;
  MMFM_REQUIRE(ws != nullptr, "mmfm_gemm_wgrad_det: null workspace");
  if (int rc = det_ws_check(ws->buf, ws->bytes, ws->tickets, ws->n_tickets, wgrad_det_need(R, NO, KI),
                            "mmfm_gemm_wgrad_det"))
    return rc;
  CUtensorMap tmY, tmX;
  int rc = make_tmap_bf16_2d(&tmY, dY, (uint64_t)R, (uint64_t)NO, (uint64_t)lddy, 64, kBK, TMA_SW_128);
  if (rc) return rc;
  rc = make_tmap_bf16_2d(&tmX, X, (uint64_t)R, (uint64_t)KI, (uint64_t)ldx, 64, kBK, TMA_SW_128);
  if (rc) return rc;
  constexpr size_t smem = (size_t)STAGES * ((2 + BN / 64) * 64 * kBK * 2) + 2048 + 1024;
  static bool attr_set = false;
  if (!attr_set) {
    MMFM_CHECK_CUDA(cudaFuncSetAttribute(gemm_wgrad_kernel<STAGES, BN, true>,
                                         cudaFuncAttributeMaxDynamicSharedMemorySize, (int)smem));
    attr_set = true;
  }
  int rows_per_split = 0;
  const int splits = wgrad_splits(R, NO, KI, BN, &rows_per_split);
  MMFM_CHECK_CUDA(launch_pdl(gemm_wgrad_kernel<STAGES, BN, true>, dim3((KI + BN - 1) / BN, (NO + kBM - 1) / kBM, splits),
                             dim3(kGemmThreads), smem, st, tmY, tmX, R, NO, KI, dW, ldw, rows_per_split, dbias, 1, 1,
                             (float4*)ws->buf, ws->tickets));
  return 0;
}

static DetNeed colsum_det_need(int R, int NO) {
  const long long slices = (NO + 511) / 512, parts = (R + kColsumRows - 1) / kColsumRows;
  return DetNeed{slices * parts * 512 * 4, (int)(slices * parts)};
}

namespace mmfm {
bool det_need_gemm(int kind, long long d0, long long d1, long long d2, DetNeed* need) {
  if (kind == MMFM_DET_WGRAD) *need = wgrad_det_need((int)d0, (int)d1, (int)d2);
  else if (kind == MMFM_DET_COLSUM) *need = colsum_det_need((int)d0, (int)d1);
  else return false;
  return true;
}
}


extern "C" int mmfm_gemm_wgrad(const void* dY, long long lddy, const void* X, long long ldx, int R, int NO, int KI,
                               float* dW, long long ldw, float* dbias, void* stream) {
  MMFM_REQUIRE(dY && X && dW, "mmfm_gemm_wgrad: null operand");
  MMFM_REQUIRE(R > 0 && NO > 0 && KI > 0, "mmfm_gemm_wgrad: bad shape R=%d NO=%d KI=%d", R, NO, KI);
  static int bn_env = -1;
  if (bn_env < 0) {
    const char* e = getenv("MMFM_WGRAD_BN");
    bn_env = e ? atoi(e) : 128;
  }
  if (bn_env == 256 && KI % 256 == 0) return launch_wgrad<256>(dY, lddy, X, ldx, R, NO, KI, dW, ldw, dbias, stream);
  return launch_wgrad<128>(dY, lddy, X, ldx, R, NO, KI, dW, ldw, dbias, stream);
}

extern "C" int mmfm_gemm_wgrad_det(const void* dY, long long lddy, const void* X, long long ldx, int R, int NO, int KI,
                                   float* dW, long long ldw, float* dbias, const mmfm_det_ws* ws, void* stream) {
  MMFM_REQUIRE(dY && X && dW, "mmfm_gemm_wgrad_det: null operand");
  MMFM_REQUIRE(R > 0 && NO > 0 && KI > 0, "mmfm_gemm_wgrad_det: bad shape R=%d NO=%d KI=%d", R, NO, KI);
  return launch_wgrad_det(dY, lddy, X, ldx, R, NO, KI, dW, ldw, dbias, ws, (cudaStream_t)stream);
}

extern "C" int mmfm_colsum_bf16(const void* dY, long long ld, int R, int NO, float* out, void* stream) {
  MMFM_REQUIRE(dY && out && R > 0 && NO > 0, "mmfm_colsum_bf16: bad arguments");
  dim3 grid((NO + 511) / 512, (R + kColsumRows - 1) / kColsumRows);
  colsum_bf16_kernel<<<grid, 256, 0, (cudaStream_t)stream>>>((const bf16*)dY, ld, R, NO, out, nullptr, nullptr);
  MMFM_CHECK_CUDA(cudaGetLastError());
  return 0;
}

extern "C" int mmfm_colsum_bf16_det(const void* dY, long long ld, int R, int NO, float* out, const mmfm_det_ws* ws,
                                    void* stream) {
  MMFM_REQUIRE(dY && out && R > 0 && NO > 0 && ws, "mmfm_colsum_bf16_det: bad arguments");
  if (int rc = det_ws_check(ws->buf, ws->bytes, ws->tickets, ws->n_tickets, colsum_det_need(R, NO), "mmfm_colsum_bf16_det"))
    return rc;
  dim3 grid((NO + 511) / 512, (R + kColsumRows - 1) / kColsumRows);
  colsum_bf16_kernel<true><<<grid, 256, 0, (cudaStream_t)stream>>>((const bf16*)dY, ld, R, NO, out, (float*)ws->buf,
                                                                   ws->tickets);
  MMFM_CHECK_CUDA(cudaGetLastError());
  return 0;
}

extern "C" int mmfm_cast_bf16(const float* x, long long ldx, void* y, long long ldy, void* yt, long long ldyt, int R,
                              int C, void* stream) {
  MMFM_REQUIRE(x && (y || yt) && R > 0 && C > 0, "mmfm_cast_bf16: bad arguments");
  dim3 grid((C + 31) / 32, (R + 31) / 32);
// ... 6 lines not shown
```

multi_modal_foundation_model_b200/csrc/norm.cu:

```cuda
#include "common.cuh"
#include "host_util.h"
#include "../../include/mmfm_b200.h"

namespace mmfm {

constexpr int kLnWarps = 8;

MMFM_DEVINL long long ln_out_row(long long r, int modmajor_T, int S, long long BT) {
  if (modmajor_T <= 0) return r;
  const long long b = r / S;
  const int s = (int)(r - b * S);
  const int m = s / modmajor_T;
  return (long long)m * BT + b * modmajor_T + (s - m * modmajor_T);
}

template <int NV>
__global__ void __launch_bounds__(kLnWarps * 32) layernorm_fwd_kernel(const float* __restrict__ x,
                                                                       const float* __restrict__ gamma,
                                                                       const float* __restrict__ beta,
                                                                       bf16* __restrict__ y, float* __restrict__ mean,
                                                                       float* __restrict__ rstd, int R, int H,
                                                                       float eps, int modmajor_T, int S) {
  pdl_enter();
  const int warp = threadIdx.x >> 5, lane = threadIdx.x & 31;
  const long long BT = modmajor_T > 0 ? (long long)(R / S) * modmajor_T : 0;
  const float invH = 1.0f / (float)H;
  if constexpr (NV > 0 && NV <= 4) {
    constexpr int U = NV <= 2 ? 4 : 2;
    for (long long r0 = ((long long)blockIdx.x * kLnWarps + warp) * U; r0 < R; r0 += (long long)gridDim.x * kLnWarps * U) {
      float4 v[U][NV];
#pragma unroll
      for (int u = 0; u < U; ++u)
#pragma unroll
        for (int j = 0; j < NV; ++j)
          v[u][j] = (r0 + u < R) ? __ldg(reinterpret_cast<const float4*>(x + (r0 + u) * H) + lane + 32 * j)
                                 : make_float4(0.f, 0.f, 0.f, 0.f);
      float mu[U], rs[U];
#pragma unroll
      for (int u = 0; u < U; ++u) {
        float s = 0.f;
#pragma unroll
        for (int j = 0; j < NV; ++j) s += (v[u][j].x + v[u][j].y) + (v[u][j].z + v[u][j].w);
        mu[u] = warp_sum(s) * invH;
        float q = 0.f;
#pragma unroll
        for (int j = 0; j < NV; ++j) {
          const float a = v[u][j].x - mu[u], b = v[u][j].y - mu[u], c = v[u][j].z - mu[u], d = v[u][j].w - mu[u];
          q += (a * a + b * b) + (c * c + d * d);
        }
        rs[u] = rsqrtf(warp_sum(q) * invH + eps);
      }
      float4 gm[NV], bt[NV];
#pragma unroll
      for (int j = 0; j < NV; ++j) {
        gm[j] = __ldg(reinterpret_cast<const float4*>(gamma) + lane + 32 * j);
        bt[j] = __ldg(reinterpret_cast<const float4*>(beta) + lane + 32 * j);
      }
#pragma unroll
      for (int u = 0; u < U; ++u) {
        const long long r = r0 + u;
        if (r >= R) break;
        if (lane == 0) {
          mean[r] = mu[u];
          rstd[r] = rs[u];
        }
        bf16* yr = y + ln_out_row(r, modmajor_T, S, BT) * H;
#pragma unroll
        for (int j = 0; j < NV; ++j) {
          uint2 o;
          o.x = pack_bf16x2((v[u][j].x - mu[u]) * rs[u] * gm[j].x + bt[j].x, (v[u][j].y - mu[u]) * rs[u] * gm[j].y + bt[j].y);
          o.y = pack_bf16x2((v[u][j].z - mu[u]) * rs[u] * gm[j].z + bt[j].z, (v[u][j].w - mu[u]) * rs[u] * gm[j].w + bt[j].w);
          reinterpret_cast<uint2*>(yr)[lane + 32 * j] = o;
        }
      }
    }
  } else {
  for (long long r = (long long)blockIdx.x * kLnWarps + warp; r < R; r += (long long)gridDim.x * kLnWarps) {
    const float* xr = x + r * H;
    bf16* yr = y + ln_out_row(r, modmajor_T, S, BT) * H;
    if constexpr (NV > 0) {
      float4 v[NV];
      float s = 0.f;
#pragma unroll
      for (int j = 0; j < NV; ++j) {
        v[j] = __ldg(reinterpret_cast<const float4*>(xr) + lane + 32 * j);
        s += (v[j].x + v[j].y) + (v[j].z + v[j].w);
      }
      const float mu = warp_sum(s) * invH;
      float q = 0.f;
#pragma unroll
      for (int j = 0; j < NV; ++j) {
        const float a = v[j].x - mu, b = v[j].y - mu, c = v[j].z - mu, d = v[j].w - mu;
        q += (a * a + b * b) + (c * c + d * d);
      }
      const float rs = rsqrtf(warp_sum(q) * invH + eps);
      if (lane == 0) {
        mean[r] = mu;
        rstd[r] = rs;
      }
#pragma unroll
      for (int j = 0; j < NV; ++j) {
        const float4 g = __ldg(reinterpret_cast<const float4*>(gamma) + lane + 32 * j);
        const float4 b = __ldg(reinterpret_cast<const float4*>(beta) + lane + 32 * j);
        uint2 o;
        o.x = pack_bf16x2((v[j].x - mu) * rs * g.x + b.x, (v[j].y - mu) * rs * g.y + b.y);
        o.y = pack_bf16x2((v[j].z - mu) * rs * g.z + b.z, (v[j].w - mu) * rs * g.w + b.w);
        reinterpret_cast<uint2*>(yr)[lane + 32 * j] = o;
      }
    } else {
      float s = 0.f;
      for (int c = lane * 4; c < H; c += 128) {
        const float4 t = __ldg(reinterpret_cast<const float4*>(xr + c));
        s += (t.x + t.y) + (t.z + t.w);
      }
      const float mu = warp_sum(s) * invH;
      float q = 0.f;
      for (int c = lane * 4; c < H; c += 128) {
        const float4 t = __ldg(reinterpret_cast<const float4*>(xr + c));
        const float a = t.x - mu, b = t.y - mu, cc = t.z - mu, d = t.w - mu;
        q += (a * a + b * b) + (cc * cc + d * d);
      }
      const float rs = rsqrtf(warp_sum(q) * invH + eps);
      if (lane == 0) {
        mean[r] = mu;
        rstd[r] = rs;
      }
      for (int c = lane * 4; c < H; c += 128) {
        const float4 t = __ldg(reinterpret_cast<const float4*>(xr + c));
        const float4 g = __ldg(reinterpret_cast<const float4*>(gamma + c));
        const float4 b = __ldg(reinterpret_cast<const float4*>(beta + c));
        uint2 o;
        o.x = pack_bf16x2((t.x - mu) * rs * g.x + b.x, (t.y - mu) * rs * g.y + b.y);
        o.y = pack_bf16x2((t.z - mu) * rs * g.z + b.z, (t.w - mu) * rs * g.w + b.w);
        *reinterpret_cast<uint2*>(yr + c) = o;
      }
    }
  }
  }
}

template <int NV, bool DET = false>
__global__ void __launch_bounds__(kLnWarps * 32) layernorm_bwd_kernel(
    const bf16* __restrict__ dy, const float* __restrict__ x, const float* __restrict__ mean,
    const float* __restrict__ rstd, const float* __restrict__ gamma, const float* dres, float* dx,
    bf16* __restrict__ dxb, DropCfg drop, float* __restrict__ dgamma, float* __restrict__ dbeta, int R, int H,
    int modmajor_T, int S, float* __restrict__ ws, unsigned int* tickets) {
  static_assert(NV > 0, "register path only");
  pdl_enter();
  __shared__ float red[kLnWarps][NV * 128 + 4];
  const int warp = threadIdx.x >> 5, lane = threadIdx.x & 31;
  const long long BT = modmajor_T > 0 ? (long long)(R / S) * modmajor_T : 0;
  const float invH = 1.0f / (float)H;
  unsigned long long seed = 0ull;
  if (drop.thresh != 0u) seed = *drop.seed;
  const uint32_t gpr = (uint32_t)((H + 15) >> 4);

  float4 gam[NV], accg[NV], accb[NV];
#pragma unroll
  for (int j = 0; j < NV; ++j) {
    gam[j] = __ldg(reinterpret_cast<const float4*>(gamma) + lane + 32 * j);
    accg[j] = make_float4(0.f, 0.f, 0.f, 0.f);
    accb[j] = make_float4(0.f, 0.f, 0.f, 0.f);
  }
  for (long long r = (long long)blockIdx.x * kLnWarps + warp; r < R; r += (long long)gridDim.x * kLnWarps) {
    const float* xr = x + r * H;
    const bf16* dyr = dy + ln_out_row(r, modmajor_T, S, BT) * H;
    const float mu = __ldg(mean + r), rs = __ldg(rstd + r);
// ... 631 lines not shown
```

multi_modal_foundation_model_b200/engine.py:

```python
from __future__ import annotations

import ctypes as C
import os
import weakref
from typing import Any, Dict, List, Optional, Tuple

import numpy as np
import torch

from . import adapter, masker as _masker, ops
from ._lib import (ACT_DGELU, ACT_DSOFTSIGN, ACT_GELU, ACT_GELU_DG, ACT_MULAUX, ACT_NONE, ACT_ROWDOT_DROP, ACT_SOFTSIGN, LOSS_CE, LOSS_MSE, LOSS_POISSON, MASK_CAUSAL,
                   MASK_KEY, MASK_KEY_OR_DIAG, CastItem, MmfmError, lib)
from .ops import NO_DROP, DropSpec

bf16 = torch.bfloat16
SMALL_C = 8

SITE_EMBED, SITE_ATTN_PROB, SITE_ATTN_OUT, SITE_XATTN_PROB, SITE_XATTN_OUT, SITE_MLP = 0, 1, 2, 3, 4, 5
SIDE_ENC, SIDE_DEC = 0, 1


def site_id(kind: int, layer: int, side: int) -> int:
    return kind + 16 * layer + 4096 * side

# ... 279 lines not shown
        self.mask = {m.name: i64(B, T) for m in mods}
        self.seed = eng.seed
        self.gscale = torch.ones(1, device=dev, dtype=torch.float32)
        self.sample_thresh = torch.zeros(len(mods), device=dev, dtype=torch.int32)
        self._thresh_host = torch.zeros(len(mods), dtype=torch.int32).pin_memory()
        self._thresh_cur = [0] * len(mods)
        self._mask_host = {m.name: torch.zeros(B, T, dtype=torch.int64).pin_memory() for m in mods}
        self.zero, self.kvalid, self.tmask = u8(S), u8(B, S), u8(B, S)
        self.nex, self.inv_n = i64(len(mods)), f32(1)
        self.mod_ids = torch.repeat_interleave(torch.tensor([m.index for m in mods], dtype=torch.int16), T).to(dev)
        self.preds = {m.name: f32(B, T, m.C) for m in mods}
        self.n_partials = 2 * max(1, lib().mmfm_sm_count())
        self.partials = torch.zeros(len(mods) * self.n_partials, device=dev)
        self.mod_loss, self.loss = f32(len(mods)), f32(1)

        rec_f, rec_b = ops.Recorder(), ops.Recorder()
        ops.set_recorder(rec_f)
        try:
            self._build_forward(f32, b16)
            ops.set_recorder(rec_b)
            self._build_backward(f32, b16)
        finally:
            ops.set_recorder(None)
        self._g_fwd = self._g_bwd = None
        self._n_fwd_runs = self._n_bwd_runs = 0
        self.fwd_calls, self.bwd_calls = rec_f.calls, rec_b.calls
        self._keep += rec_f.keep + rec_b.keep
        if self.det_ws is not None:
            self.det_ws.materialize(dev)
        self.n_fwd, self.n_bwd = len(self.fwd_calls), len(self.bwd_calls)

    def _drop(self, kind: int, layer: int, side: int, p: float) -> DropSpec:
        if not self.training or p <= 0.0:
            return NO_DROP
        return DropSpec(self.seed, site_id(kind, layer, side), p)

    def _ln_fwd(self, x, name, y, stats, modmajor=False):
        st = self.eng.store
        mean, rstd = torch.empty(self.R, device=x.device), torch.empty(self.R, device=x.device)
        self._keep += [mean, rstd]
        stats[name] = (mean, rstd)
        if st.has(name + ".scale"):
            assert not modmajor
            ops.scalenorm_fwd(x, st.p(name + ".scale"), y, rstd, R=self.R, H=self.eng.H)
            return
        ops.layernorm_fwd(x, st.p(name + ".weight"), st.p(name + ".bias"), y, mean, rstd, R=self.R, H=self.eng.H,
                          modmajor_T=self.eng.T if modmajor else 0, S=self.S if modmajor else 0)

    def _ln_bwd(self, dy, x, name, dres, dx, dxb, drop, modmajor=False):
        st = self.eng.store
        mean, rstd = self.stats[name]
        if st.has(name + ".scale"):
            ops.scalenorm_bwd(dy, x, rstd, st.p(name + ".scale"), dres, dx, dxb, drop, st.g(name + ".scale"), R=self.R,
                              H=self.eng.H, ws=self.det_ws)
            return
        ops.layernorm_bwd(dy, x, mean, rstd, st.p(name + ".weight"), dres, dx, dxb, drop, st.g(name + ".weight"),
                          st.g(name + ".bias"), R=self.R, H=self.eng.H, modmajor_T=self.eng.T if modmajor else 0,
                          S=self.S if modmajor else 0, ws=self.det_ws)

    def _bias(self, names: List[str], buf: str = "p") -> Optional[torch.Tensor]:
        st = self.eng.store
        if not st.has(names[0]):
            return None
        base = st.flat if buf == "p" else st.grad
        o0 = st.offset[st.alias[names[0]]]
        n = 0
        for nm in names:
            assert st.offset[st.alias[nm]] == o0 + n, "fused biases must be adjacent in the flat buffer"
            n += st.shape[nm].numel()
            assert st.shape[nm].numel() % 64 == 0 or nm == names[-1], "fused biases need 64-element multiples"
        return base[o0:o0 + n]

    def _wgrad_dst(self, names: List[str]) -> torch.Tensor:
        st = self.eng.store
        o0 = st.offset[names[0]]
        n = 0
        for nm in names:
            assert st.offset[nm] == o0 + n, "fused weights must be adjacent in the flat buffer"
            n += st.shape[nm].numel()
            assert len(names) == 1 or st.shape[nm].numel() % 64 == 0
        cols = st.shape[names[0]][1]
        return st.grad[o0:o0 + n].view(n // cols, cols)

    def _attention(self, fwd: bool, tag: str, q, k, v, o, mode, nh, p_drop, kind_p, kind_o, layer, side, sep,
                   grads=None, prep_done=False):
        B, S, H = self.B, self.S, self.eng.H
        d = H // nh
        if fwd:
            self.lse[tag] = torch.empty(B, nh, S, device=q.device)
            dp = self._drop(kind_p, layer, side, p_drop)
            if dp.thresh:
                self.pkeep[tag] = torch.zeros(B * nh * S * ((S + 63) // 64) * 4, device=q.device, dtype=torch.int16)
        dp = self._drop(kind_p, layer, side, p_drop)
        do = self._drop(kind_o, layer, side, p_drop)
        kw = dict(B=B, n_heads=nh, Sq=S, Sk=S, d_head=d, mask_mode=mode, mod_q=self.mod_ids if sep else None,
                  mod_k=self.mod_ids if sep else None, drop_p=dp, drop_o=do, p_keep=self.pkeep.get(tag))
        if fwd:
            ops.attention_fwd(q, k, v, o, self.lse[tag], self.kvalid, **kw)
        else:
            d_o, dq, dk, dv = grads
            ops.attention_bwd(q, k, v, o, self.lse[tag], self.kvalid, d_o=d_o, delta=self.delta, dq=dq, dk=dk, dv=dv,
                              prep_done=prep_done, **kw)

    def _build_forward(self, f32, b16):
        eng = self.eng
        st, sh, mods = eng.store, eng.shadows, self.mods
        B, T, H, S, R, BT = self.B, eng.T, eng.H, self.S, self.R, self.BT
        self.stats: Dict[str, Tuple[torch.Tensor, torch.Tensor]] = {}
        self.lse: Dict[str, torch.Tensor] = {}
        self.pkeep: Dict[str, torch.Tensor] = {}
        self.act: Dict[str, torch.Tensor] = {}
        A = self.act

        sh.refresh()
        ops.mask_prep([self.mask[m.name] for m in mods], [self.attn[m.name] for m in mods], [m.C for m in mods],
                      self.zero, self.kvalid, self.tmask, self.nex, self.inv_n, sample_thresh=self.sample_thresh,
                      seed=self.seed)

        self.emb = {SIDE_ENC: f32(R, H), SIDE_DEC: f32(R, H)}
        self.xs = [f32(R, H)]
        self.ys = [f32(R, H)]
        self.inb: Dict[str, torch.Tensor] = {}
        for side, sname, x0, p_emb in ((SIDE_ENC, "encoder_embeddings", self.xs[0], eng.hp["embed_dropout"]),
                                       (SIDE_DEC, "decoder_embeddings", self.ys[0], eng.hp["dec_embed_dropout"])):
            for k, m in enumerate(mods):
                pre = f"{self.prefix}{sname}.{m.name}.embedder"
                off = k * T
                pos = st.p(pre + ".pos_embed.weight") if st.has(pre + ".pos_embed.weight") else None
                ops.embed_assemble(st.p(pre + ".mod_emb.weight")[m.index], pos, self.ts[m.name], self.emb[side], B=B,
                                   T=T, S=S, off=off, H=H)
                drop = self._drop(SITE_EMBED, m.index, side, p_emb)
                b1 = st.p(pre + ".token_embed.bias") if st.has(pre + ".token_embed.bias") else None
                if m.small:
                    A[pre + ".hid"] = f32(BT, 2 * m.C)
                    ops.smallc_embed_fwd(self.inp[m.name], st.p(pre + ".token_embed.weight"), b1,
                                         st.p(pre + ".projection.weight"), st.p(pre + ".projection.bias"),
                                         self.emb[side], x0, A[pre + ".hid"], self.zero, drop, eng.embed_scale,
                                         eng.embed_act, B=B, T=T, S=S, off=off, Cc=m.C, H=H)
                else:
                    if m.name not in self.inb:
                        self.inb[m.name] = b16(BT, m.C)
                        if m.name in self.u8_mods:
                            ops.u8_expand(self.inp_u8[m.name].view(BT, m.C), None, self.inb[m.name], R=BT, Cc=m.C)
                            ops.u8_expand(self.tgt_u8[m.name].view(BT, m.C), self.tgt[m.name].view(BT, m.C), None,
                                          R=BT, Cc=m.C)
                        else:
                            ops.cast_bf16(self.inp[m.name].view(BT, m.C), self.inb[m.name])
                    A[pre + ".hid"] = b16(BT, 2 * m.C)
                    ops.gemm_tn(self.inb[m.name], sh.nat[pre + ".token_embed"], A[pre + ".hid"], bias=b1,
                                act=eng.embed_act, act_scale=eng.embed_scale)
                    ops.gemm_tn(A[pre + ".hid"], sh.nat[pre + ".projection"], x0, bias=st.p(pre + ".projection.bias"),
                                drop=drop, remap=(T, S, off), row_zero=self.zero, res=self.emb[side])

        def attn_block(pre, x_in, x_out, ln_name, mode, nh, p_drop, layer, side, sep):
            A[ln_name] = b16(R, H)
            self._ln_fwd(x_in, ln_name, A[ln_name], self.stats)
            A[pre + ".qkv"] = b16(R, 3 * H)
            ops.gemm_tn(A[ln_name], sh.nat[pre + ".qkv"], A[pre + ".qkv"],
                        bias=self._bias([f"{pre}.{k}.bias" for k in ("query", "key", "value")]))
            qkv = A[pre + ".qkv"]
            A[pre + ".ao"] = b16(R, H)
            self._attention(True, pre, qkv[:, :H], qkv[:, H:2 * H], qkv[:, 2 * H:], A[pre + ".ao"], mode, nh, p_drop,
                            SITE_ATTN_PROB, SITE_ATTN_OUT, layer, side, sep)
            ops.gemm_tn(A[pre + ".ao"], sh.nat[pre + ".out_proj"], x_out, bias=self._bias([pre + ".out_proj.bias"]),
                        res=x_in)

        def mlp_block(pre, x_in, x_out, ln_name, p_drop, layer, side, inter):
            A[ln_name] = b16(R, H)
            self._ln_fwd(x_in, ln_name, A[ln_name], self.stats)
            A[pre + ".dg"], A[pre + ".g"] = b16(R, inter), b16(R, inter)
            ops.gemm_tn(A[ln_name], sh.nat[pre + ".up_proj"], A[pre + ".g"], bias=self._bias([pre + ".up_proj.bias"]),
                        act=ACT_GELU_DG if eng.save_gelu_grad else ACT_GELU, D2=A[pre + ".dg"])
            ops.gemm_tn(A[pre + ".g"], sh.nat[pre + ".down_proj"], x_out, bias=self._bias([pre + ".down_proj.bias"]),
                        drop=self._drop(SITE_MLP, layer, side, p_drop), res=x_in)

        hp = eng.hp
        for i in range(eng.Le):
            pre = f"encoder.{i}"
            self.xs += [f32(R, H), f32(R, H)]
            attn_block(pre + ".attn", self.xs[2 * i], self.xs[2 * i + 1], pre + ".ln1", MASK_KEY_OR_DIAG,
                       hp["enc_heads"], hp["enc_dropout"], i, SIDE_ENC, False)
            mlp_block(pre + ".mlp", self.xs[2 * i + 1], self.xs[2 * i + 2], pre + ".ln2", hp["enc_dropout"], i,
                      SIDE_ENC, eng.enc_inter)
        A["encoder_norm"] = b16(R, H)
        self._ln_fwd(self.xs[-1], "encoder_norm", A["encoder_norm"], self.stats)
        self.ctx = f32(R, H)
        ops.gemm_tn(A["encoder_norm"], sh.nat["decoder_proj_context"], self.ctx,
                    bias=st.p("decoder_proj_context.bias"), res=self.emb[SIDE_ENC])

        dec_mode = MASK_CAUSAL if eng.causal else MASK_KEY
        if eng.fuse_ctx:
            names = [f"decoder.{i}.context_norm" for i in range(eng.Ld)]
            for n in names:
                A[n] = b16(R, H)
            cmean, crstd = torch.empty(R, device=self.ctx.device), torch.empty(R, device=self.ctx.device)
            self._keep += [cmean, crstd]
            for n in names:
                self.stats[n] = (cmean, crstd)
            ops.layernorm_fwd_multi(self.ctx, [st.p(n + ".weight") for n in names], [st.p(n + ".bias") for n in names],
                                    [A[n] for n in names], cmean, crstd, R=R, H=H)
        for i in range(eng.Ld):
            pre = f"decoder.{i}"
            self.ys += [f32(R, H), f32(R, H), f32(R, H)]
            y0, y1, y2, y3 = self.ys[3 * i: 3 * i + 4]
            attn_block(pre + ".attn", y0, y1, pre + ".ln1", dec_mode, hp["dec_heads"], hp["dec_dropout"], i, SIDE_DEC,
                       eng.sep)
            xa = pre + ".cross_attn"
            A[pre + ".query_norm"] = b16(R, H)
            self._ln_fwd(y1, pre + ".query_norm", A[pre + ".query_norm"], self.stats)
            if not eng.fuse_ctx:
                A[pre + ".context_norm"] = b16(R, H)
                self._ln_fwd(self.ctx, pre + ".context_norm", A[pre + ".context_norm"], self.stats)
            A[xa + ".q"], A[xa + ".kv"] = b16(R, H), b16(R, 2 * H)
            ops.gemm_tn(A[pre + ".query_norm"], sh.nat[xa + ".query"], A[xa + ".q"], bias=self._bias([xa + ".query.bias"]))
            ops.gemm_tn(A[pre + ".context_norm"], sh.nat[xa + ".kv"], A[xa + ".kv"],
                        bias=self._bias([xa + ".key.bias", xa + ".value.bias"]))
            A[xa + ".ao"] = b16(R, H)
            self._attention(True, xa, A[xa + ".q"], A[xa + ".kv"][:, :H], A[xa + ".kv"][:, H:], A[xa + ".ao"],
                            MASK_KEY_OR_DIAG, hp["dec_heads"], hp["dec_dropout"], SITE_XATTN_PROB, SITE_XATTN_OUT, i,
                            SIDE_DEC, False)
            ops.gemm_tn(A[xa + ".ao"], sh.nat[xa + ".out_proj"], y2, bias=self._bias([xa + ".out_proj.bias"]), res=y1)
            mlp_block(pre + ".mlp", y2, y3, pre + ".ln2", hp["dec_dropout"], i, SIDE_DEC, eng.dec_inter)
        A["decoder_norm"] = b16(R, H)
        self._ln_fwd(self.ys[-1], "decoder_norm", A["decoder_norm"], self.stats, modmajor=True)

        self.dpreds: Dict[str, torch.Tensor] = {}
        for k, m in enumerate(mods):
            pre = f"{self.prefix}decoder_embeddings.{m.name}.out"
            ym = A["decoder_norm"][k * BT:(k + 1) * BT]
            pr = self.preds[m.name].view(BT, m.C)
            if m.small:
                ops.smallc_head_fwd(ym, st.p(pre + ".weight"), st.p(pre + ".bias"), pr, R=BT, H=H, Cc=m.C)
            else:
                ops.gemm_tn(ym, sh.nat[pre], pr, bias=st.p(pre + ".bias"))
            self.dpreds[m.name] = b16(BT, m.C)
            ops.loss_fwd_bwd(pr, self.tgt[m.name].view(BT, m.C), self.tmask, self.inv_n, m.loss_kind,
                             self.partials[k * self.n_partials:(k + 1) * self.n_partials], self.dpreds[m.name], B=B,
                             T=T, Cc=m.C, S=S, off=k * T)
        ops.loss_finalize(self.partials, self.n_partials, len(mods), self.inv_n, self.mod_loss, self.loss)

    def _build_backward(self, f32, b16):
        eng = self.eng
        st, sh, mods, hp = eng.store, eng.shadows, self.mods, eng.hp
        B, T, H, S, R, BT = self.B, eng.T, eng.H, self.S, self.R, self.BT
        A = self.act
        G, Genc, Gctx = f32(R, H), f32(R, H), f32(R, H)
        Gb, Gcb = b16(R, H), b16(R, H)
        d_ao, dh = b16(R, H), b16(R, H)
        dqkv = b16(R, 3 * H)
        du = b16(R, max(eng.enc_inter, eng.dec_inter))
        self.delta = f32(B, max(hp["enc_heads"], hp["dec_heads"]), S)
        ddec = b16(R, H)
        self.grad_marks: List[Tuple[int, int]] = []

        def mark(next_param: Optional[str]):
            rec = ops._REC
            off = st.total if next_param is None else st.offset[st.alias[next_param]]
            self.grad_marks.append((len(rec.calls), off))

        def lin_bwd(dY, X, wname, shadow_key, dX, *, act=ACT_NONE, aux=None, act_scale=1.0, wnames=None, bnames=None,
                    **extra):
            if dX is not None:
                ops.gemm_tn(dY, sh.tr[shadow_key], dX, act=act, aux=aux, act_scale=act_scale, **extra)
            bn = bnames or [wname + ".bias"]
            ops.gemm_wgrad(dY, X, self._wgrad_dst(wnames or [wname + ".weight"]),
                           dbias=self._bias(bn, "g") if st.has(bn[0]) else None, ws=self.det_ws)

        def mlp_bwd(pre, x_in, ln_name, Gs, inter, dxb, drop_prev):
            duv = du[:, :inter]
            lin_bwd(Gb, A[pre + ".g"], pre + ".down_proj", pre + ".down_proj", duv,
                    act=ACT_MULAUX if eng.save_gelu_grad else ACT_DGELU, aux=A[pre + ".dg"])
            lin_bwd(duv, A[ln_name], pre + ".up_proj", pre + ".up_proj", dh)
            self._ln_bwd(dh, x_in, ln_name, Gs, Gs, dxb, drop_prev)

        def out_proj_bwd(pre, nh, p_drop, kind_o, layer, side):
            fuse = eng.fuse_attn_prep and H // nh == 32
            if fuse:
                lin_bwd(Gb, A[pre + ".ao"], pre + ".out_proj", pre + ".out_proj", d_ao, act=ACT_ROWDOT_DROP,
                        aux=A[pre + ".ao"], rowdot=self.delta, rowdot_S=S, drop=self._drop(kind_o, layer, side, p_drop))
            else:
                lin_bwd(Gb, A[pre + ".ao"], pre + ".out_proj", pre + ".out_proj", d_ao)
            return fuse

        def attn_bwd(pre, x_in, ln_name, Gs, mode, nh, p_drop, layer, side, sep, dxb, drop_prev):
            fused = out_proj_bwd(pre, nh, p_drop, SITE_ATTN_OUT, layer, side)
            qkv = A[pre + ".qkv"]
            self._attention(False, pre, qkv[:, :H], qkv[:, H:2 * H], qkv[:, 2 * H:], A[pre + ".ao"], mode, nh, p_drop,
                            SITE_ATTN_PROB, SITE_ATTN_OUT, layer, side, sep,
                            grads=(d_ao, dqkv[:, :H], dqkv[:, H:2 * H], dqkv[:, 2 * H:]), prep_done=fused)
            lin_bwd(dqkv, A[ln_name], None, pre + ".qkv", dh,
                    wnames=[f"{pre}.{k}.weight" for k in ("query", "key", "value")],
                    bnames=[f"{pre}.{k}.bias" for k in ("query", "key", "value")])
            self._ln_bwd(dh, x_in, ln_name, Gs, Gs, dxb, drop_prev)

        for k, m in reversed(list(enumerate(mods))):
            pre = f"{self.prefix}decoder_embeddings.{m.name}.out"
            ym = A["decoder_norm"][k * BT:(k + 1) * BT]
            dym = ddec[k * BT:(k + 1) * BT]
            if m.small:
                ops.smallc_head_bwd(ym, st.p(pre + ".weight"), self.dpreds[m.name], dym, st.g(pre + ".weight"),
                                    st.g(pre + ".bias"), R=BT, H=H, Cc=m.C, ws=self.det_ws)
            else:
                lin_bwd(self.dpreds[m.name], ym, pre, pre, dym)
        last_dec_drop = self._drop(SITE_MLP, eng.Ld - 1, SIDE_DEC, hp["dec_dropout"])
        self._ln_bwd(ddec, self.ys[-1], "decoder_norm", None, G, Gb, last_dec_drop, modmajor=True)

        dec_mode = MASK_CAUSAL if eng.causal else MASK_KEY
        dqx, dkvx = b16(R, H), b16(R, 2 * H)
        dctx: List[torch.Tensor] = []
        for i in reversed(range(eng.Ld)):
            pre = f"decoder.{i}"
            y0, y1, y2, y3 = self.ys[3 * i: 3 * i + 4]
            mlp_bwd(pre + ".mlp", y2, pre + ".ln2", G, eng.dec_inter, Gb, NO_DROP)
            xa = pre + ".cross_attn"
            fused = out_proj_bwd(xa, hp["dec_heads"], hp["dec_dropout"], SITE_XATTN_OUT, i, SIDE_DEC)
            self._attention(False, xa, A[xa + ".q"], A[xa + ".kv"][:, :H], A[xa + ".kv"][:, H:], A[xa + ".ao"],
                            MASK_KEY_OR_DIAG, hp["dec_heads"], hp["dec_dropout"], SITE_XATTN_PROB, SITE_XATTN_OUT, i,
                            SIDE_DEC, False, grads=(d_ao, dqx, dkvx[:, :H], dkvx[:, H:]), prep_done=fused)
            lin_bwd(dqx, A[pre + ".query_norm"], xa + ".query", xa + ".query", dh)
            self._ln_bwd(dh, y1, pre + ".query_norm", G, G, Gb, NO_DROP)
            if eng.fuse_ctx:
                dctx.append(b16(R, H))
                lin_bwd(dkvx, A[pre + ".context_norm"], None, xa + ".kv", dctx[-1],
                        wnames=[xa + ".key.weight", xa + ".value.weight"], bnames=[xa + ".key.bias", xa + ".value.bias"])
            else:
                lin_bwd(dkvx, A[pre + ".context_norm"], None, xa + ".kv", dh,
                        wnames=[xa + ".key.weight", xa + ".value.weight"], bnames=[xa + ".key.bias", xa + ".value.bias"])
                first = i == eng.Ld - 1
                self._ln_bwd(dh, self.ctx, pre + ".context_norm", None if first else Gctx, Gctx, Gcb if i == 0 else None,
                             NO_DROP)
            prev = self._drop(SITE_MLP, i - 1, SIDE_DEC, hp["dec_dropout"]) if i > 0 else NO_DROP
            attn_bwd(pre + ".attn", y0, pre + ".ln1", G, dec_mode, hp["dec_heads"], hp["dec_dropout"], i, SIDE_DEC,
                     eng.sep, Gb if i > 0 else None, prev)
            if i > 0:
                mark(f"decoder.{i - 1}.mlp.down_proj.weight")
            elif eng.fuse_ctx:
                mark(f"decoder.{eng.Ld - 1}.context_norm.weight")
        if eng.fuse_ctx:
            names = [f"decoder.{i}.context_norm" for i in reversed(range(eng.Ld))]
            cmean, crstd = self.stats[names[0]]
            ops.layernorm_bwd_multi(dctx, self.ctx, cmean, crstd, [st.p(n + ".weight") for n in names], Gctx, Gcb,
                                    [st.g(n + ".weight") for n in names], [st.g(n + ".bias") for n in names], R=R, H=H,
                                    ws=self.det_ws)
        mark("decoder_proj_context.weight")

        lin_bwd(Gcb, A["encoder_norm"], "decoder_proj_context", "decoder_proj_context", dh)
        last_enc_drop = self._drop(SITE_MLP, eng.Le - 1, SIDE_ENC, hp["enc_dropout"])
        self._ln_bwd(dh, self.xs[-1], "encoder_norm", None, Genc, Gb, last_enc_drop)
        for i in reversed(range(eng.Le)):
            pre = f"encoder.{i}"
            mlp_bwd(pre + ".mlp", self.xs[2 * i + 1], pre + ".ln2", Genc, eng.enc_inter, Gb, NO_DROP)
            prev = self._drop(SITE_MLP, i - 1, SIDE_ENC, hp["enc_dropout"]) if i > 0 else NO_DROP
            attn_bwd(pre + ".attn", self.xs[2 * i], pre + ".ln1", Genc, MASK_KEY_OR_DIAG, hp["enc_heads"],
                     hp["enc_dropout"], i, SIDE_ENC, False, Gb if i > 0 else None, prev)
            if i > 0:
                mark(f"encoder.{i - 1}.mlp.down_proj.weight")

        dtok = b16(BT, H)
        for side, sname, Gs, G2, p_emb in ((SIDE_DEC, "decoder_embeddings", G, None, hp["dec_embed_dropout"]),
                                           (SIDE_ENC, "encoder_embeddings", Genc, Gctx, hp["embed_dropout"])):
            for k, m in reversed(list(enumerate(mods))):
                pre = f"{self.prefix}{sname}.{m.name}.embedder"
                off = k * T
                dpos = st.g(pre + ".pos_embed.weight") if st.has(pre + ".pos_embed.weight") else None
                ops.embed_assemble_bwd(Gs, G2, self.ts[m.name], dpos, st.g(pre + ".mod_emb.weight")[m.index], B=B, T=T,
                                       S=S, off=off, H=H, ws=self.det_ws)
                drop = self._drop(SITE_EMBED, m.index, side, p_emb)
                if m.small:
                    has_b1 = st.has(pre + ".token_embed.bias")
                    db1 = st.g(pre + ".token_embed.bias") if has_b1 else f32(2 * m.C)
                    ops.smallc_embed_bwd(self.inp[m.name], A[pre + ".hid"], st.p(pre + ".projection.weight"), Gs,
                                         self.zero, drop, eng.embed_scale, eng.embed_act,
                                         st.g(pre + ".token_embed.weight"), db1, st.g(pre + ".projection.weight"),
                                         st.g(pre + ".projection.bias"), B=B, T=T, S=S, off=off, Cc=m.C, H=H,
                                         ws=self.det_ws)
                else:
                    ops.embed_grad_prep(Gs, dtok, self.zero, drop, B=B, T=T, S=S, off=off, H=H)
                    dhid = b16(BT, 2 * m.C)
                    back = ACT_DSOFTSIGN if eng.embed_act == ACT_SOFTSIGN else ACT_NONE
                    lin_bwd(dtok, A[pre + ".hid"], pre + ".projection", pre + ".projection", dhid, act=back,
                            aux=A[pre + ".hid"] if back else None, act_scale=eng.embed_scale)
                    lin_bwd(dhid, self.inb[m.name], pre + ".token_embed", None, None)
        mark(None)
        ops.scale_inplace(st.grad, self.gscale)

    def _fwd_body(self):
        self.seed.add_(0x632BE59BD9B4E019)
        ops.run_recorded(self.fwd_calls)

    def set_sample_thresh(self, thresh: List[int]) -> None:
        if thresh != self._thresh_cur:
            for k, v in enumerate(thresh):
                self._thresh_host[k] = v - (1 << 32) if v >= (1 << 31) else v
            self.sample_thresh.copy_(self._thresh_host, non_blocking=True)
            self._thresh_cur = list(thresh)

    def _bwd_body(self):
        self.eng.store.grad.zero_()
        ops.run_recorded(self.bwd_calls)

    def _capture(self, body):
        g = torch.cuda.CUDAGraph()
        with torch.cuda.graph(g):
            body()
        return g

    def run_forward(self):
        if self.eng.use_graphs and self._g_fwd is None and self._n_fwd_runs >= 1:
            self._g_fwd = self._capture(self._fwd_body)
        self._n_fwd_runs += 1
        if self._g_fwd is not None:
            self._g_fwd.replay()
        else:
            self._fwd_body()

    def run_backward(self):
        if self.eng.use_graphs and self._g_bwd is None and self._n_bwd_runs >= 1:
            self._g_bwd = self._capture(self._bwd_body)
        self._n_bwd_runs += 1
        if self._g_bwd is not None:
            self._g_bwd.replay()
        else:
            self._bwd_body()


class _StepFn(torch.autograd.Function):

    @staticmethod
    def forward(ctx, anchor, eng, plan):
        plan.run_forward()
        ctx.eng, ctx.plan = eng, plan
        return plan.loss.clone().reshape(())

    @staticmethod
    def backward(ctx, grad_loss):
        ctx.eng.backward(ctx.plan, grad_loss)
        return None, None, None


class Engine:
    _created = 0

    def __init__(self, model):
        self.model = model
        p0 = next(model.parameters())
        if p0.device.type != "cuda":
            raise MmfmError("the B200 path runs on a CUDA device only (move the model with .cuda() / .to('cuda') "
                            "first); there is no CPU fallback")
        lib()
        self.device = p0.device
        groups = embedding_groups(model)
        hp = adapter.hyper_params(model, groups)
        self.hp = hp
        loss_kind = adapter.loss_kinds(model)
        self.H = model.hidden_size
        self.Le, self.Ld = model.n_enc_layers, model.n_dec_layers
        self.fuse_ctx = fuse_context_norms(dict(model.named_parameters(remove_duplicate=False)), self.Ld)
        self.causal, self.sep = bool(model.decoder_causal_mask), bool(model.decoder_sep_mask)
        if hp["enc_act"] != "gelu" or hp["dec_act"] != "gelu":
            raise NotImplementedError("only act='gelu' (mm.yaml:44) is built for the transformer MLP")
        act = hp["embed_act"]
        if act not in ("softsign", "identity"):
            raise NotImplementedError(f"embedder act {act!r}: only 'softsign' (mm.yaml:33) and 'identity' are built")
        self.embed_act = ACT_SOFTSIGN if act == "softsign" else ACT_NONE
        self.sessions: Dict[Any, Tuple[str, List[ModSpec]]] = {}
        self.multi_session = getattr(model, "session_embeddings", None) is not None
        for prefix, enc, dec in groups:
            names = list(dec.keys())
            if names != list(enc.keys()):
                raise NotImplementedError("encoder and decoder must embed the same modalities in the same order")
            key = prefix.split(".")[1] if self.multi_session else None
            self.sessions[key] = (prefix, [ModSpec(n, model.mod_to_indx[n], enc[n].n_channel,
                                                   loss_kind.get(n, "mse")) for n in names])
        self.mods = next(iter(self.sessions.values()))[1]
        self.embed_scale = float(hp["embed_scale"])
        if self.embed_act == ACT_NONE and self.embed_scale != 1.0:
            raise NotImplementedError("identity embedder activation needs scale == 1")
        self.enc_inter = model.encoder[0].mlp.up_proj.out_features
        self.dec_inter = model.decoder[0].mlp.up_proj.out_features
        for nh in (hp["enc_heads"], hp["dec_heads"]):
            if self.H // nh not in (32, 64):
                raise NotImplementedError(f"head size {self.H // nh}: the attention kernels are built for 32 and 64")
        self.T: Optional[int] = None
        Engine._created += 1
        key = (torch.initial_seed() * 0x9E3779B97F4A7C15 + Engine._created * 0xD1B54A32D192ED03) & 0x3FFFFFFFFFFFFFFF
        self.seed = torch.tensor([key], dtype=torch.int64, device=self.device)
        self.store = ParamStore(model, self.device)
        self.shadows = Shadows(self.store, model, self.sessions)
        self.plans: Dict[Tuple[int, bool, Any, Tuple[str, ...], bool], Plan] = {}
        self.arenas: Dict[Tuple[int, bool], Arena] = {}
        self.ddp = None
        import os as _os
        self.use_graphs = _os.environ.get("MMFM_CUDA_GRAPHS", "1") != "0"
        self.save_gelu_grad = _os.environ.get("MMFM_GELU_SAVE", "dg") != "u"
        self.fuse_attn_prep = (_os.environ.get("MMFM_FUSE_ATTN_PREP", "1") != "0" and self.H > 64 and self.H % 32 == 0
                               and _os.environ.get("MMFM_GEMM_TS", "1") != "0")
        self.last_plan: Optional[Plan] = None
        self._grad_views = None
        from .model import MultiModalOutput
        self.output_cls = MultiModalOutput

    def _plan(self, B: int, T: int, training: bool, session=None, u8_mods: Tuple[str, ...] = ()) -> Plan:
        if self.T is None:
            self.T = T
        elif self.T != T:
            self.plans.clear()
            self.arenas.clear()
            self.T = T
        key = (B, training, session, u8_mods, ops.deterministic())
        pl = self.plans.get(key)
        if pl is None:
            arena = None
            if self.multi_session:
                arena = self.arenas.get((B, training))
                if arena is None:
                    widest = max(self.sessions, key=lambda k: sum(m.C for m in self.sessions[k][1]))
                    probe = Plan(self, B, training, widest)
                    nbytes = probe.arena_bytes + (1 << 20)
                    del probe
                    arena = self.arenas[(B, training)] = Arena(nbytes, self.device)
            pl = Plan(self, B, training, session, arena, u8_mods)
            self.plans[key] = pl
        return pl

    def reseed(self, value: int) -> None:
        self.seed.fill_(int(value) & 0x3FFFFFFFFFFFFFFF)

    def step(self, mod_dict: Dict[str, Dict[str, Any]]):
        model = self.model
        MultiModalOutput = self.output_cls
        if not self.store.adopted():
            self.store.adopt()
        session = None
        if self.multi_session:
            eid = next(iter(mod_dict.values())).get("eid")
            session = model.session_key(eid)
            if session not in self.sessions:
                raise MmfmError(f"unknown session {eid!r}: the model holds {sorted(self.sessions)[:4]} ...")
        mods = self.sessions[session][1]
        names = [m.name for m in mods]
        if list(mod_dict.keys()) != names:
            raise MmfmError(f"mod_dict must hold exactly the modalities {names} in this order")
        d0 = mod_dict[names[0]]
        if d0["inputs"].dim() == 2:
            raise MmfmError("first modality must be (B,T,C)")
        B, T = d0["inputs"].shape[:2]
        training = bool(model.training)
        u8_mods = tuple(m.name for m in mods if not m.small and mod_dict[m.name]["inputs"].dtype == torch.uint8)
        for m in mods:
            if mod_dict[m.name]["inputs"].dtype == torch.uint8 and m.name not in u8_mods:
                raise MmfmError(f"modality {m.name}: uint8 inputs are only supported for spike-count modalities (C > {SMALL_C})")
        pl = self._plan(B, T, training, session, u8_mods)
        thresh = [0] * len(mods)
        for k, m in enumerate(mods):
            d = mod_dict[m.name]
            if d["inputs"].dim() == 2:
                d["inputs"] = d["inputs"].unsqueeze(-1)
                d["targets"] = d["targets"].unsqueeze(-1)
            if d.get("masking_mode"):
                raise NotImplementedError("mask_type 'input' (mm.py:256-263) is broken in the reference itself "
                                          "(UnboundLocalError at mm.py:272); only masking_mode=None is supported")
            if tuple(d["inputs"].shape) != (B, T, m.C):
                raise MmfmError(f"modality {m.name}: inputs shape {tuple(d['inputs'].shape)} != {(B, T, m.C)}")
            if m.name in u8_mods:
                if d["targets"].dtype != torch.uint8:
                    raise MmfmError(f"modality {m.name}: uint8 inputs need uint8 targets")
                pl.inp_u8[m.name].copy_(d["inputs"], non_blocking=True)
                pl.tgt_u8[m.name].copy_(d["targets"], non_blocking=True)
            else:
                pl.inp[m.name].copy_(d["inputs"], non_blocking=True)
                pl.tgt[m.name].copy_(d["targets"], non_blocking=True)
            pl.attn[m.name].copy_(d["inputs_attn_mask"], non_blocking=True)
            pl.ts[m.name].copy_(d["inputs_timestamp"], non_blocking=True)
            im = d.get("inputs_modality")
            if not (torch.is_tensor(im) and im.is_cuda) and im is not None and int(im) != m.index:
                raise MmfmError(f"modality {m.name}: inputs_modality {int(im)} != {m.index}")
            em = d.get("eval_mask")
            if em is None:
                mk = model.masker
                stream = adapter.mask_stream(model)
                if _masker.inactive(mk):
                    pl.mask[m.name].zero_()
                elif stream == "device" and _masker.device_samplable(mk):
                    thresh[k] = max(1, min(0xFFFFFFFF, int(float(mk.ratio) * 4294967296.0)))
                else:
                    regions = d.get("inputs_regions") if m.name == "ap" else None
                    col = _masker.sample_mask_column(mk, (B, T, m.C), regions,
                                                     "fast" if stream == "device" else stream)
                    hb = pl._mask_host[m.name]
                    hb.copy_(col)
                    pl.mask[m.name].copy_(hb, non_blocking=True)
            elif isinstance(em, (bool, int)):
                pl.mask[m.name].fill_(int(bool(em)))
            elif em.dim() == 2:
                pl.mask[m.name].copy_(em, non_blocking=True)
            else:
                pl.mask[m.name].copy_(em[:, :, 0], non_blocking=True)
        pl.set_sample_thresh(thresh)
        self.last_plan = pl
        anchor = None
        if torch.is_grad_enabled():
            anchor = next((p for p in self.store.params.values() if p.requires_grad), None)
        if anchor is not None:
            loss = _StepFn.apply(anchor, self, pl)
        else:
            pl.run_forward()
            loss = pl.loss.clone().reshape(())
        out_loss, out_n, out_p, out_t = {}, {}, {}, {}
        mod_loss = pl.mod_loss.clone()
        nex = pl.nex.clone()
# ... 39 lines not shown
```

multi_modal_foundation_model_b200/ops.py:

```python
from __future__ import annotations

import ctypes as C
from typing import Callable, List, Optional, Sequence, Tuple

import torch

from . import _lib
from ._lib import (ACT_DGELU, ACT_DSOFTSIGN, ACT_GELU, ACT_NONE, ACT_SOFTSIGN, LOSS_MSE, LOSS_POISSON, MASK_CAUSAL,
                   MASK_KEY, MASK_KEY_OR_DIAG, AttnArgs, CastItem, Dropout, GemmArgs, MaskArgs, check, lib)

bf16 = torch.bfloat16


def _stream() -> int:
    return torch.cuda.current_stream().cuda_stream


def _p(t: Optional[torch.Tensor]) -> Optional[int]:
    return None if t is None else t.data_ptr()


class DropSpec:

    __slots__ = ("seed", "site", "thresh", "scale")

    def __init__(self, seed: Optional[torch.Tensor], site: int, p: float):
        t = int(round(float(p) * 256.0))
        t = max(0, min(255, t))
        if seed is None:
            t = 0
        self.seed = seed
        self.site = int(site)
        self.thresh = t
        self.scale = 256.0 / (256.0 - t)

    def c(self) -> Dropout:
        return Dropout(_p(self.seed) if self.thresh else None, self.site, self.thresh, self.scale)


NO_DROP = DropSpec(None, 0, 0.0)


class Recorder:

    def __init__(self):
        self.calls: List[Tuple[Callable, tuple, str]] = []
        self.keep: List[object] = []

    def add(self, fn, args, what, meta=None):
        self.calls.append((fn, args, what, meta or {}))


_REC: Optional[Recorder] = None


def set_recorder(r: Optional[Recorder]) -> None:
    global _REC
    _REC = r


def _launch(name: str, *args, keep=(), meta=None):
    fn = getattr(lib(), name)
    if _REC is not None:
        _REC.keep.extend(keep)
        _REC.add(fn, args, name, meta)
        return
    check(fn(*args, _stream()), name)


def deterministic() -> bool:
    return torch.are_deterministic_algorithms_enabled()


def det_ws_need(kind: int, d0: int, d1: int = 1, d2: int = 0) -> Tuple[int, int]:
    nb, nt = C.c_longlong(0), C.c_int(0)
    check(lib().mmfm_det_ws_bytes(kind, int(d0), int(d1), int(d2), C.byref(nb), C.byref(nt)), "mmfm_det_ws_bytes")
    return nb.value, nt.value


class DetWorkspace:

    def __init__(self):
        self.c = _lib.DetWs(None, 0, None, 0)
        self.want_bytes, self.want_tickets = 0, 0
        self.buf: Optional[torch.Tensor] = None
        self.tickets: Optional[torch.Tensor] = None

    def require(self, nbytes: int, n_tickets: int) -> None:
        self.want_bytes = max(self.want_bytes, int(nbytes))
        self.want_tickets = max(self.want_tickets, int(n_tickets))

    def materialize(self, device) -> None:
        if self.buf is None or self.buf.numel() < self.want_bytes:
            self.buf = torch.empty(max(16, self.want_bytes), dtype=torch.uint8, device=device)
        if self.tickets is None or self.tickets.numel() < self.want_tickets:
            self.tickets = torch.zeros(max(1, self.want_tickets), dtype=torch.int32, device=device)
        self.c.buf, self.c.bytes = self.buf.data_ptr(), self.buf.numel()
        self.c.tickets, self.c.n_tickets = self.tickets.data_ptr(), self.tickets.numel()


def _launch_det(name: str, ws: Optional[DetWorkspace], need: Tuple[int, int], device, *args, keep=(), meta=None):
    if ws is None:
        ws = DetWorkspace()
    ws.require(*need)
    if _REC is None:
        ws.materialize(device)
    _launch(name + "_det", *args, C.byref(ws.c), keep=(*keep, ws), meta=meta)


def run_recorded(calls) -> None:
    st = _stream()
    for c in calls:
        rc = c[0](*c[1], st)
        if rc != 0:
            check(rc, c[2])


def count_kernels(calls) -> int:
    return sum(int(c[3].get("kernels", 1)) for c in calls)


def run_recorded_timed(calls):
    st = _stream()
    evs = [torch.cuda.Event(enable_timing=True) for _ in range(len(calls) + 1)]
    evs[0].record()
    for i, c in enumerate(calls):
        rc = c[0](*c[1], st)
        evs[i + 1].record()
        if rc != 0:
            check(rc, c[2])
    torch.cuda.synchronize()
    return [(c[2], c[3], evs[i].elapsed_time(evs[i + 1])) for i, c in enumerate(calls)]


def gemm_tn(A: torch.Tensor, B: torch.Tensor, D: torch.Tensor, *, M: Optional[int] = None, N: Optional[int] = None,
            K: Optional[int] = None, bias: Optional[torch.Tensor] = None, res: Optional[torch.Tensor] = None,
            D2: Optional[torch.Tensor] = None, aux: Optional[torch.Tensor] = None, act: int = ACT_NONE,
            act_scale: float = 1.0, drop: DropSpec = NO_DROP, remap: Tuple[int, int, int] = (0, 0, 0),
            row_zero: Optional[torch.Tensor] = None, lda: Optional[int] = None, ldb: Optional[int] = None,
            ldd: Optional[int] = None, ldr: Optional[int] = None, ldaux: Optional[int] = None,
            rowdot: Optional[torch.Tensor] = None, rowdot_S: int = 0) -> None:
    assert A.dtype == bf16 and B.dtype == bf16 and D.dtype in (bf16, torch.float32)
    a = GemmArgs()
    a.A, a.lda = A.data_ptr(), (lda if lda is not None else A.stride(0))
    a.B, a.ldb = B.data_ptr(), (ldb if ldb is not None else B.stride(0))
    a.M = M if M is not None else A.shape[0]
    a.N = N if N is not None else B.shape[0]
    a.K = K if K is not None else A.shape[1]
    a.D, a.ldd = D.data_ptr(), (ldd if ldd is not None else D.stride(0))
    a.d_fp32 = 1 if D.dtype == torch.float32 else 0
    a.D2 = _p(D2)
    if bias is not None:
        assert bias.dtype == torch.float32
    a.bias = _p(bias)
    if res is not None:
        assert res.dtype == torch.float32
    a.res, a.ldr = _p(res), (ldr if ldr is not None else (res.stride(0) if res is not None else 0))
    a.aux, a.ldaux = _p(aux), (ldaux if ldaux is not None else (aux.stride(0) if aux is not None else 0))
    a.act, a.act_scale = act, act_scale
    a.drop = drop.c()
    a.remap_T, a.remap_S, a.remap_off = remap
    a.row_zero = _p(row_zero)
    if rowdot is not None:
        assert rowdot.dtype == torch.float32 and rowdot_S > 0
    a.rowdot, a.rowdot_S = _p(rowdot), int(rowdot_S)
    mn = float(a.M) * a.N
    nbytes = 2.0 * a.M * a.K + 2.0 * a.N * a.K + mn * (4 if a.d_fp32 else 2)
    nbytes += (2.0 * mn if D2 is not None else 0.0) + (4.0 * mn if res is not None else 0.0) + (2.0 * mn if aux is not None else 0.0)
    _launch("mmfm_gemm_tn", C.byref(a), keep=(a,),
            meta={"flops": 2.0 * a.M * a.N * a.K, "bytes": nbytes, "tag": f"gemm_tn {a.M}x{a.N}x{a.K}"})


def gemm_wgrad(dY: torch.Tensor, X: torch.Tensor, dW: torch.Tensor, *, R: Optional[int] = None,
               NO: Optional[int] = None, KI: Optional[int] = None, ldw: Optional[int] = None,
               dbias: Optional[torch.Tensor] = None, ws: Optional[DetWorkspace] = None) -> None:
    assert dY.dtype == bf16 and X.dtype == bf16 and dW.dtype == torch.float32
    R = R if R is not None else dY.shape[0]
    NO = NO if NO is not None else dY.shape[1]
    KI = KI if KI is not None else X.shape[1]
    args = (dY.data_ptr(), dY.stride(0), X.data_ptr(), X.stride(0), R, NO, KI, dW.data_ptr(),
            ldw if ldw is not None else KI, _p(dbias))
    meta = {"flops": 2.0 * R * NO * KI, "bytes": 2.0 * R * (NO + KI) + 4.0 * NO * KI, "tag": f"wgrad {R}x{NO}x{KI}"}
    if deterministic():
        _launch_det("mmfm_gemm_wgrad", ws, det_ws_need(_lib.DET_WGRAD, R, NO, KI), dW.device, *args, meta=meta)
        return
    _launch("mmfm_gemm_wgrad", *args, meta=meta)


def colsum_bf16(dY: torch.Tensor, out: torch.Tensor, *, R: Optional[int] = None, NO: Optional[int] = None,
                ws: Optional[DetWorkspace] = None) -> None:
    R = R if R is not None else dY.shape[0]
    NO = NO if NO is not None else dY.shape[1]
    args = (dY.data_ptr(), dY.stride(0), R, NO, out.data_ptr())
    if deterministic():
        _launch_det("mmfm_colsum_bf16", ws, det_ws_need(_lib.DET_COLSUM, R, NO), out.device, *args)
        return
    _launch("mmfm_colsum_bf16", *args)


def cast_bf16(x: torch.Tensor, y: Optional[torch.Tensor], yt: Optional[torch.Tensor] = None, *, R: Optional[int] = None,
              Cc: Optional[int] = None, ldx: Optional[int] = None) -> None:
    assert x.dtype == torch.float32
    R = R if R is not None else x.shape[0]
    Cc = Cc if Cc is not None else x.shape[1]
    _launch("mmfm_cast_bf16", x.data_ptr(), ldx if ldx is not None else x.stride(0), _p(y),
            y.stride(0) if y is not None else 0, _p(yt), yt.stride(0) if yt is not None else 0, R, Cc,
            meta={"bytes": float(R) * Cc * (4 + 2 * (y is not None) + 2 * (yt is not None))})


def cast_bf16_multi(items_dev: torch.Tensor, n_items: int, total_tiles: int) -> None:
    _launch("mmfm_cast_bf16_multi", items_dev.data_ptr(), n_items, total_tiles)


def scale_inplace(x: torch.Tensor, scale_dev: torch.Tensor) -> None:
    _launch("mmfm_scale_inplace", x.data_ptr(), x.numel(), scale_dev.data_ptr())


def csr_to_dense_u8(data: torch.Tensor, indices: torch.Tensor, row_ptr: torch.Tensor, out: torch.Tensor, *,
                    n_rows: int, n_cols: int) -> None:
    assert out.dtype == torch.uint8 and out.is_contiguous() and out.numel() == n_rows * n_cols
    _launch("mmfm_csr_to_dense_u8", _p(data) if data.numel() else None, _p(indices) if indices.numel() else None,
            row_ptr.data_ptr(), n_rows, n_cols, out.data_ptr(), meta={"bytes": float(n_rows) * n_cols + 5.0 * data.numel()})


def u8_expand(x: torch.Tensor, y32: Optional[torch.Tensor], y16: Optional[torch.Tensor], *, R: int, Cc: int) -> None:
    assert x.dtype == torch.uint8 and x.is_contiguous()
    _launch("mmfm_u8_expand", x.data_ptr(), R, Cc, _p(y32), y32.stride(0) if y32 is not None else 0, _p(y16),
            y16.stride(0) if y16 is not None else 0, meta={"bytes": float(R) * Cc * (1 + (4 if y32 is not None else 0) + (2 if y16 is not None else 0))})


def column_stats(pred: torch.Tensor, y: torch.Tensor, out: torch.Tensor, *, log_rate: bool,
                 ws: Optional[DetWorkspace] = None) -> None:
    R, Cc = pred.shape
    args = (pred.data_ptr(), y.data_ptr(), R, Cc, 1 if log_rate else 0, out.data_ptr())
    if deterministic():
        _launch_det("mmfm_column_stats", ws, det_ws_need(_lib.DET_COLUMN_STATS, R, Cc), out.device, *args,
                    meta={"bytes": 8.0 * R * Cc})
        return
    _launch("mmfm_column_stats", *args, meta={"bytes": 8.0 * R * Cc})


def adamw_step(p: torch.Tensor, g: torch.Tensor, exp_avg: torch.Tensor, exp_avg_sq: torch.Tensor, *, lr: float,
               beta1: float, beta2: float, eps: float, weight_decay: float, step: int) -> None:
    n = p.numel()
    _launch("mmfm_adamw_step", p.data_ptr(), g.data_ptr(), exp_avg.data_ptr(), exp_avg_sq.data_ptr(), n, float(lr),
            float(beta1), float(beta2), float(eps), float(weight_decay), int(step), meta={"bytes": 28.0 * n})


def layernorm_fwd(x, gamma, beta, y, mean, rstd, *, R: int, H: int, eps: float = 1e-5, modmajor_T: int = 0,
                  S: int = 0) -> None:
    _launch("mmfm_layernorm_fwd", x.data_ptr(), gamma.data_ptr(), beta.data_ptr(), y.data_ptr(), mean.data_ptr(),
            rstd.data_ptr(), R, H, eps, modmajor_T, S, meta={"bytes": 6.0 * R * H})


def layernorm_bwd(dy, x, mean, rstd, gamma, dres, dx, dxb, drop: DropSpec, dgamma, dbeta, *, R: int, H: int,
                  modmajor_T: int = 0, S: int = 0, ws: Optional[DetWorkspace] = None) -> None:
    d = drop.c()
    args = (dy.data_ptr(), x.data_ptr(), mean.data_ptr(), rstd.data_ptr(), gamma.data_ptr(), _p(dres), _p(dx), _p(dxb),
            C.byref(d), _p(dgamma), _p(dbeta), R, H, modmajor_T, S)
    meta = {"bytes": float(R) * H * (2 + 4 + (4 if dres is not None else 0) + (4 if dx is not None else 0)
                                     + (2 if dxb is not None else 0))}
    if deterministic():
        _launch_det("mmfm_layernorm_bwd", ws, det_ws_need(_lib.DET_LN_BWD, R, H), x.device, *args, keep=(d,), meta=meta)
        return
    _launch("mmfm_layernorm_bwd", *args, keep=(d,), meta=meta)


def layernorm_fwd_multi(x, gammas, betas, ys, mean, rstd, *, R: int, H: int, eps: float = 1e-5) -> None:
    a = _lib.LnMultiArgs()
    a.x, a.R, a.H, a.n, a.eps = x.data_ptr(), R, H, len(ys), eps
    for l, (g, b, y) in enumerate(zip(gammas, betas, ys)):
        a.gamma[l], a.beta[l], a.y[l] = g.data_ptr(), b.data_ptr(), y.data_ptr()
    a.mean, a.rstd = mean.data_ptr(), rstd.data_ptr()
    _launch("mmfm_layernorm_fwd_multi", C.byref(a), keep=(a,), meta={"bytes": float(R) * H * (4 + 2 * len(ys))})


def layernorm_bwd_multi(dys, x, mean, rstd, gammas, dx, dxb, dgammas, dbetas, *, R: int, H: int,
                        ws: Optional[DetWorkspace] = None) -> None:
    a = _lib.LnMultiArgs()
    a.x, a.R, a.H, a.n, a.eps = x.data_ptr(), R, H, len(dys), 0.0
    for l, (dy, g, dg, db) in enumerate(zip(dys, gammas, dgammas, dbetas)):
        a.dy[l], a.gamma[l], a.dgamma[l], a.dbeta[l] = dy.data_ptr(), g.data_ptr(), _p(dg), _p(db)
    a.mean, a.rstd, a.dx, a.dxb = mean.data_ptr(), rstd.data_ptr(), dx.data_ptr(), _p(dxb)
    meta = {"bytes": float(R) * H * (4 + 2 * len(dys) + 4 + (2 if dxb is not None else 0))}
    if deterministic():
        _launch_det("mmfm_layernorm_bwd_multi", ws, det_ws_need(_lib.DET_LN_BWD_MULTI, R, H, len(dys)), x.device,
                    C.byref(a), keep=(a,), meta=meta)
        return
    _launch("mmfm_layernorm_bwd_multi", C.byref(a), keep=(a,), meta=meta)


def scalenorm_fwd(x, g, y, rnorm, *, R: int, H: int, eps: float = 1e-5) -> None:
    _launch("mmfm_scalenorm_fwd", x.data_ptr(), g.data_ptr(), y.data_ptr(), rnorm.data_ptr(), R, H, eps,
            meta={"bytes": 6.0 * R * H})


def scalenorm_bwd(dy, x, rnorm, g, dres, dx, dxb, drop: DropSpec, dg, *, R: int, H: int, eps: float = 1e-5,
                  ws: Optional[DetWorkspace] = None) -> None:
    d = drop.c()
    args = (dy.data_ptr(), x.data_ptr(), rnorm.data_ptr(), g.data_ptr(), _p(dres), _p(dx), _p(dxb), C.byref(d), _p(dg),
            R, H, eps)
    meta = {"bytes": float(R) * H * (2 + 4 + (4 if dres is not None else 0) + (4 if dx is not None else 0)
                                     + (2 if dxb is not None else 0))}
    if deterministic():
        _launch_det("mmfm_scalenorm_bwd", ws, det_ws_need(_lib.DET_SCALENORM_BWD, R, H), x.device, *args, keep=(d,),
                    meta=meta)
        return
    _launch("mmfm_scalenorm_bwd", *args, keep=(d,), meta=meta)


def _attn_args(q, k, v, o, lse, key_valid, *, B, n_heads, Sq, Sk, d_head, mask_mode, mod_q=None, mod_k=None,
               drop_p: DropSpec = NO_DROP, drop_o: DropSpec = NO_DROP, p_keep=None, d_o=None, delta=None, dq=None,
               dk=None, dv=None, prep_done: bool = False) -> AttnArgs:
    a = AttnArgs()
    a.q, a.ldq = q.data_ptr(), q.stride(0)
    a.k, a.ldk = k.data_ptr(), k.stride(0)
    a.v, a.ldv = v.data_ptr(), v.stride(0)
    a.o, a.ldo = o.data_ptr(), o.stride(0)
    a.lse = lse.data_ptr()
    a.key_valid = key_valid.data_ptr()
    a.mod_q, a.mod_k = _p(mod_q), _p(mod_k)
    a.B, a.n_heads, a.Sq, a.Sk, a.d_head = B, n_heads, Sq, Sk, d_head
    a.mask_mode = mask_mode
# ... 117 lines not shown
```

Baseline: 26470.

## Fuse the following LayerNorm into the residual GEMM epilogue for H=256

Adds a GEMM variant whose epilogue applies bias, dropout and the residual add, writes the fp32 residual stream, then computes LayerNorm over both 128-column tiles of a row. It emits the bf16 normalized output plus mean/rstd. Each CTA owns both N tiles of a row block, so the pre-norm row is staged in extra TMEM. This removes separate LayerNorm launches and their re-read of the fp32 residual in the forward pass. In exchange it doubles TMEM use, adds named barriers, and ties the path to H == 256.

```diff
diff --git a/include/mmfm_b200.h b/include/mmfm_b200.h
--- a/include/mmfm_b200.h
+++ b/include/mmfm_b200.h
@@ -8,7 +8,7 @@
 extern "C" {
 #endif
 
-#define MMFM_ABI_VERSION 5
+#define MMFM_ABI_VERSION 6
 
 const char* mmfm_last_error(void);
 int mmfm_abi_version(void);
@@ -50,6 +50,17 @@
 } mmfm_gemm_args;
 
 int mmfm_gemm_tn(const mmfm_gemm_args* args, void* stream);
+
+typedef struct mmfm_ln_epi {
+  const float* gamma;
+  const float* beta;
+  void* y;
+  float* mean;
+  float* rstd;
+  float eps;
+  int modmajor_T, S;
+} mmfm_ln_epi;
+int mmfm_gemm_tn_ln(const mmfm_gemm_args* args, const mmfm_ln_epi* ln, void* stream);
 
 int mmfm_gemm_wgrad(const void* dY, long long lddy, const void* X, long long ldx, int R, int NO, int KI, float* dW,
                     long long ldw, float* dbias, void* stream);
diff --git a/multi_modal_foundation_model_b200/_lib.py b/multi_modal_foundation_model_b200/_lib.py
--- a/multi_modal_foundation_model_b200/_lib.py
+++ b/multi_modal_foundation_model_b200/_lib.py
@@ -14,7 +14,7 @@
               "-Xptxas", "-v"]
 
 MAX_MOD = 8
-ABI_VERSION = 5
+ABI_VERSION = 6
 MASK_SITE = 8192
 
 
@@ -84,6 +84,13 @@
     ]
 
 
+class LnEpi(C.Structure):
+    _fields_ = [
+        ("gamma", C.c_void_p), ("beta", C.c_void_p), ("y", C.c_void_p), ("mean", C.c_void_p), ("rstd", C.c_void_p),
+        ("eps", C.c_float), ("modmajor_T", C.c_int), ("S", C.c_int),
+    ]
+
+
 class AttnArgs(C.Structure):
     _fields_ = [
         ("q", C.c_void_p), ("ldq", C.c_longlong),
@@ -156,6 +163,7 @@
 
 SIGNATURES = {
     "mmfm_gemm_tn": [C.POINTER(GemmArgs), _vp],
+    "mmfm_gemm_tn_ln": [C.POINTER(GemmArgs), C.POINTER(LnEpi), _vp],
     "mmfm_gemm_wgrad": [_vp, _ll, _vp, _ll, _i, _i, _i, _vp, _ll, _vp, _vp],
     "mmfm_colsum_bf16": [_vp, _ll, _i, _i, _vp, _vp],
     "mmfm_cast_bf16": [_vp, _ll, _vp, _ll, _vp, _ll, _i, _i, _vp],
diff --git a/multi_modal_foundation_model_b200/csrc/common.cuh b/multi_modal_foundation_model_b200/csrc/common.cuh
--- a/multi_modal_foundation_model_b200/csrc/common.cuh
+++ b/multi_modal_foundation_model_b200/csrc/common.cuh
@@ -337,6 +337,19 @@
 #pragma unroll
   for (int o = 16; o > 0; o >>= 1) v += __shfl_xor_sync(0xffffffffu, v, o);
   return v;
+}
+
+MMFM_DEVINL void named_bar_sync(uint32_t id, uint32_t threads) {
+  asm volatile("bar.sync %0, %1;" ::"r"(id), "r"(threads) : "memory");
+}
+
+template <typename I>
+MMFM_DEVINL I ln_out_row(I r, int modmajor_T, int S, I BT) {
+  if (modmajor_T <= 0) return r;
+  const I b = r / S;
+  const int s = (int)(r - b * S);
+  const int m = s / modmajor_T;
+  return (I)m * BT + b * modmajor_T + (s - m * modmajor_T);
 }
 
 MMFM_DEVINL uint32_t pack_bf16x2(float lo, float hi) {
diff --git a/multi_modal_foundation_model_b200/csrc/gemm.cu b/multi_modal_foundation_model_b200/csrc/gemm.cu
--- a/multi_modal_foundation_model_b200/csrc/gemm.cu
+++ b/multi_modal_foundation_model_b200/csrc/gemm.cu
@@ -59,21 +59,26 @@
   EPI_DSOFTSIGN = 6,
   EPI_GENERIC = 7,
   EPI_GELU_DG = 8,
-  EPI_MULAUX = 9
+  EPI_MULAUX = 9,
+  EPI_RES_F32_LN = 10
 };
 
 template <int BN, int STAGES, int EPI>
 __global__ void __launch_bounds__(kTnThreads, 1) gemm_tn_kernel(const __grid_constant__ CUtensorMap tmA,
                                                                  const __grid_constant__ CUtensorMap tmB,
                                                                  const mmfm_gemm_args p, int tiles_n, int n_tiles,
-                                                                 int bstat) {
+                                                                 int bstat, const mmfm_ln_epi ln) {
   constexpr uint32_t kABytes = kBM * kBK * 2;
   constexpr uint32_t kBBytes = BN * kBK * 2;
   constexpr uint32_t kStageBytes = kABytes + kBBytes;
-  constexpr uint32_t kTmemCols = 2 * BN;
+  constexpr uint32_t kTmemCols = (EPI == EPI_RES_F32_LN ? 4 : 2) * BN;
   constexpr int kPitch = BN + 4;
   constexpr int kHalf = BN / (kEpiWarps / 4);
   constexpr bool GEN = EPI == EPI_GENERIC;
+  constexpr int NU = EPI == EPI_RES_F32_LN ? 2 : 1;
+  auto sched = [&](int k) {
+    return NU == 1 ? (int)blockIdx.x + k * (int)gridDim.x : ((int)blockIdx.x + (k / NU) * (int)gridDim.x) * NU + k % NU;
+  };
 
   constexpr int kMaxStages = 8;
   extern __shared__ uint8_t smem_raw[];
@@ -130,10 +135,10 @@
         mbar_arrive_expect_tx(&b_full, b_res_bytes);
         for (int kb = 0; kb < nkb; ++kb) tma_load_2d_addr(smem_base + kb * kBBytes, &tmB, &b_full, kb * kBK, n0);
       }
-      for (int tile = blockIdx.x; tile < n_tiles; tile += gridDim.x) {
+      for (int k = 0, tile; (tile = sched(k)) < n_tiles; ++k) {
         const int m0 = (tile / tiles_n) * kBM, n0 = (tile % tiles_n) * BN;
         {
-          const int t2 = tile + 2 * (int)gridDim.x;
+          const int t2 = sched(k + 2);
           if (t2 < n_tiles && (t2 % tiles_n == 0 || tiles_n > (int)gridDim.x)) {
             const int m2 = (t2 / tiles_n) * kBM;
             for (int kb = 0; kb < nkb; ++kb) tma_prefetch_l2_2d(&tmA, kb * kBK, m2);
@@ -154,7 +159,7 @@
       const uint32_t idesc = make_idesc_bf16(kBM, BN, 0, 0);
       uint32_t it = 0, t = 0;
       if (bstat) mbar_wait(&b_full, 0);
-      for (int tile = blockIdx.x; tile < n_tiles; tile += gridDim.x, ++t) {
+      for (; sched((int)t) < n_tiles; ++t) {
         const uint32_t buf = t & 1u;
         if (t >= 2) mbar_wait(&acc_empty[buf], ((t >> 1) - 1) & 1);
         tc_fence_after();
@@ -174,6 +179,148 @@
           umma_commit(&empty_bar[s]);
         }
         umma_commit(&acc_full[buf]);
+      }
+    }
+  } else if constexpr (EPI == EPI_RES_F32_LN) {
+    static_assert(BN == 128 && kHalf == 32 && NU == 2, "the LayerNorm epilogue is built for H = 2 x 128");
+    constexpr int H = NU * BN;
+    const int ew = warp - 2;
+    const int quad = warp & 3;
+    const int slice = ew >> 2;
+    const int cbase = slice * kHalf;
+    const int row_l = quad * 32 + lane;
+    const int rb_row = quad * 32 + slice * 8;
+    const bool drop = p.drop.thresh != 0u;
+    const unsigned long long seed = drop ? *p.drop.seed : 0ull;
+    const uint32_t drop_gpr = (uint32_t)((p.N + 15) >> 4);
+    const uint32_t qbar = 1u + (uint32_t)quad;
+    const float invH = 1.0f / (float)H;
+    const int BT = ln.modmajor_T > 0 ? (p.M / ln.S) * ln.modmajor_T : 0;
+    __shared__ __align__(16) float s_vec[3 * H];
+    for (int i = threadIdx.x - 64; i < 3 * H; i += kEpiWarps * 32)
+      s_vec[i] = i < H ? (p.bias ? __ldg(p.bias + i) : 0.f) : __ldg(i < 2 * H ? ln.gamma + (i - H) : ln.beta + (i - 2 * H));
+    named_bar_sync(5, kEpiWarps * 32);
+    const float* s_gamma = s_vec + H;
+    const float* s_beta = s_vec + 2 * H;
+    const float* src_b = stage_f + rb_row * kPitch + lane * 4;
+    const uint32_t x_tmem = tmem_base + ((uint32_t)(quad * 32) << 16) + 2u * BN + (uint32_t)(slice * 32);
+    uint32_t t = 0;
+    for (int rb = blockIdx.x; rb * NU < n_tiles; rb += gridDim.x) {
+      const int m0 = rb * kBM;
+      const int r = m0 + row_l;
+      const int rows = min(8, p.M - (m0 + rb_row));
+      const int g0 = m0 + rb_row;
+#pragma unroll
+      for (int hh = 0; hh < NU; ++hh, ++t) {
+        const uint32_t buf = t & 1u;
+        const int n0 = hh * BN;
+        const float* bias_s = s_vec + n0 + cbase;
+        if (r < p.M)
+          asm volatile("prefetch.global.L2 [%0];" ::"l"(p.res + (long long)r * p.ldr + n0 + cbase));
+        __syncwarp();
+        mbar_wait(&acc_full[buf], (t >> 1) & 1);
+        tc_fence_after();
+        const uint32_t t_row = tmem_base + buf * BN + ((uint32_t)(quad * 32) << 16) + (uint32_t)cbase;
+        float* my_row = stage_f + row_l * kPitch + cbase;
+#pragma unroll
+        for (int c0 = 0; c0 < 32; c0 += 16) {
+          uint32_t acc[16];
+          tmem_ld16(t_row + (uint32_t)c0, acc);
+          tmem_ld_wait();
+          float v[16];
+#pragma unroll
+          for (int j4 = 0; j4 < 4; ++j4) {
+            const float4 b4 = *reinterpret_cast<const float4*>(bias_s + c0 + j4 * 4);
+            v[4 * j4 + 0] = __uint_as_float(acc[4 * j4 + 0]) + b4.x;
+            v[4 * j4 + 1] = __uint_as_float(acc[4 * j4 + 1]) + b4.y;
+            v[4 * j4 + 2] = __uint_as_float(acc[4 * j4 + 2]) + b4.z;
+            v[4 * j4 + 3] = __uint_as_float(acc[4 * j4 + 3]) + b4.w;
+          }
+          if (drop) {
+            const uint4 w = drop_bytes16(seed, p.drop.site, (uint64_t)r, drop_gpr, (uint32_t)((n0 + cbase + c0) >> 4));
+#pragma unroll
+            for (int j = 0; j < 16; ++j) v[j] = (drop_byte(w, j) < p.drop.thresh) ? 0.f : v[j] * p.drop.scale;
+          }
+#pragma unroll
+          for (int j4 = 0; j4 < 4; ++j4)
+            *reinterpret_cast<float4*>(my_row + c0 + j4 * 4) =
+                make_float4(v[4 * j4], v[4 * j4 + 1], v[4 * j4 + 2], v[4 * j4 + 3]);
+        }
+        tc_fence_before();
+        __syncwarp();
+        if (lane == 0) mbar_arrive(&acc_empty[buf]);
+        named_bar_sync(qbar, 128);
+        const float4* rsrc = reinterpret_cast<const float4*>(p.res + (long long)g0 * p.ldr + n0) + lane;
+        float4* dst = reinterpret_cast<float4*>(reinterpret_cast<float*>(p.D) + (long long)g0 * p.ldd + n0) + lane;
+        const int ldr4 = (int)(p.ldr >> 2), ldd4 = (int)(p.ldd >> 2);
+#pragma unroll
+        for (int q2 = 0; q2 < 2; ++q2) {
+          float4 xv[4];
+#pragma unroll
+          for (int j = 0; j < 4; ++j)
+            if (4 * q2 + j < rows) xv[j] = __ldg(rsrc + (4 * q2 + j) * ldr4);
+          uint32_t w[16];
+#pragma unroll
+          for (int j = 0; j < 4; ++j) {
+            if (4 * q2 + j < rows) {
+              const float4 v = *reinterpret_cast<const float4*>(src_b + (4 * q2 + j) * kPitch);
+              xv[j] = make_float4(v.x + xv[j].x, v.y + xv[j].y, v.z + xv[j].z, v.w + xv[j].w);
+              dst[(4 * q2 + j) * ldd4] = xv[j];
+            }
+            w[4 * j] = __float_as_uint(xv[j].x); w[4 * j + 1] = __float_as_uint(xv[j].y);
+            w[4 * j + 2] = __float_as_uint(xv[j].z); w[4 * j + 3] = __float_as_uint(xv[j].w);
+          }
+          tmem_st16(x_tmem + (uint32_t)(hh * BN) + 16u * q2, w);
+        }
+        named_bar_sync(qbar, 128);
+        tmem_st_wait();
+      }
+#pragma unroll
+      for (int q2 = 0; q2 < 2; ++q2) {
+        if (4 * q2 >= rows) break;
+        float4 xv[NU][4];
+#pragma unroll
+        for (int hh = 0; hh < NU; ++hh) {
+          uint32_t w[16];
+          tmem_ld16(x_tmem + (uint32_t)(hh * BN) + 16u * q2, w);
+          tmem_ld_wait();
+#pragma unroll
+          for (int j = 0; j < 4; ++j)
+            xv[hh][j] = make_float4(__uint_as_float(w[4 * j]), __uint_as_float(w[4 * j + 1]),
+                                    __uint_as_float(w[4 * j + 2]), __uint_as_float(w[4 * j + 3]));
+        }
+#pragma unroll
+        for (int j = 0; j < 4; ++j) {
+          if (4 * q2 + j >= rows) break;
+          const int gr = g0 + 4 * q2 + j;
+          float s = 0.f;
+#pragma unroll
+          for (int hh = 0; hh < NU; ++hh) s += (xv[hh][j].x + xv[hh][j].y) + (xv[hh][j].z + xv[hh][j].w);
+          const float mu = warp_sum(s) * invH;
+          float q = 0.f;
+#pragma unroll
+          for (int hh = 0; hh < NU; ++hh) {
+            const float a = xv[hh][j].x - mu, b = xv[hh][j].y - mu, c = xv[hh][j].z - mu, d = xv[hh][j].w - mu;
+            q += (a * a + b * b) + (c * c + d * d);
+          }
+          const float rs = rsqrtf(warp_sum(q) * invH + ln.eps);
+          if (lane == 0) {
+            ln.mean[gr] = mu;
+            ln.rstd[gr] = rs;
+          }
+          uint2* yr = reinterpret_cast<uint2*>(reinterpret_cast<bf16*>(ln.y) +
+                                               (long long)ln_out_row(gr, ln.modmajor_T, ln.S, BT) * H);
+#pragma unroll
+          for (int hh = 0; hh < NU; ++hh) {
+            const float4 x = xv[hh][j];
+            const float4 g = reinterpret_cast<const float4*>(s_gamma)[lane + 32 * hh];
+            const float4 b = reinterpret_cast<const float4*>(s_beta)[lane + 32 * hh];
+            uint2 o;
+            o.x = pack_bf16x2((x.x - mu) * rs * g.x + b.x, (x.y - mu) * rs * g.y + b.y);
+            o.y = pack_bf16x2((x.z - mu) * rs * g.z + b.z, (x.w - mu) * rs * g.w + b.w);
+            yr[lane + 32 * hh] = o;
+          }
+        }
       }
     }
   } else {
@@ -214,7 +361,7 @@
     for (int tile = blockIdx.x; tile < n_tiles; tile += gridDim.x, ++t) {
       const uint32_t buf = t & 1u;
       const int m0 = (tile / tiles_n) * kBM, n0 = (tile % tiles_n) * BN;
-      const long long r = (long long)m0 + row_l;
+      const int r = m0 + row_l;
       const bool warp_has_cols = (n0 + cbase) < p.N;
       if (lane < kHalf) my_bias[lane] = bias_next[0];
       if (lane + 32 < kHalf) my_bias[lane + 32] = bias_next[1];
@@ -734,7 +881,7 @@
 using namespace mmfm;
 
 template <int BN, int STAGES, int EPI>
-static int launch_tn(const mmfm_gemm_args* a, cudaStream_t st) {
+static int launch_tn(const mmfm_gemm_args* a, cudaStream_t st, const mmfm_ln_epi* ln = nullptr) {
   CUtensorMap tmA, tmB;
   int rc = make_tmap_bf16_2d(&tmA, a->A, (uint64_t)a->M, (uint64_t)a->K, (uint64_t)a->lda, kBK, kBM, TMA_SW_128);
   if (rc) return rc;
@@ -757,16 +904,23 @@
   }
   const int nkb = (a->K + kBK - 1) / kBK;
   int bstat = 0;
-  if (bstat_env && (size_t)nkb * BN * kBK * 2 * 2 <= (size_t)STAGES * (kBM * kBK * 2 + BN * kBK * 2) &&
+  if (EPI != EPI_RES_F32_LN && bstat_env && (size_t)nkb * BN * kBK * 2 * 2 <= (size_t)STAGES * (kBM * kBK * 2 + BN * kBK * 2) &&
       tiles_n <= device_sm_count() && tiles_m > 1) {
     int per_n = device_sm_count() / tiles_n;
     if (per_n > tiles_m) per_n = tiles_m;
     grid = per_n * tiles_n;
     bstat = 1;
   }
-  set_l2_window(a->D, (size_t)a->M * (size_t)a->ldd * (a->d_fp32 ? 4 : 2));
+  mmfm_ln_epi lnv = {};
+  if (EPI == EPI_RES_F32_LN) {
+    lnv = *ln;
+    grid = tiles_m < device_sm_count() ? tiles_m : device_sm_count();
+    set_l2_window(ln->y, (size_t)a->M * (size_t)a->N * 2);
+  } else {
+    set_l2_window(a->D, (size_t)a->M * (size_t)a->ldd * (a->d_fp32 ? 4 : 2));
+  }
   MMFM_CHECK_CUDA(launch_pdl(gemm_tn_kernel<BN, STAGES, EPI>, dim3(grid), dim3(kTnThreads), smem, st, tmA, tmB, *a, tiles_n,
-                             n_tiles, bstat));
+                             n_tiles, bstat, lnv));
   return 0;
 }
 
@@ -842,6 +996,28 @@
   }
 }
 
+extern "C" int mmfm_gemm_tn_ln(const mmfm_gemm_args* a, const mmfm_ln_epi* ln, void* stream) {
+  MMFM_REQUIRE(a != nullptr && ln != nullptr, "mmfm_gemm_tn_ln: null args");
+  MMFM_REQUIRE(a->M > 0 && a->K > 0, "mmfm_gemm_tn_ln: bad shape M=%d N=%d K=%d", a->M, a->N, a->K);
+  MMFM_REQUIRE(a->N == 256, "mmfm_gemm_tn_ln: the fused LayerNorm is built for N == 256 (got %d)", a->N);
+  MMFM_REQUIRE(a->A && a->B && a->D && a->res, "mmfm_gemm_tn_ln: null operand (A, B, D and res are required)");
+  MMFM_REQUIRE(a->d_fp32 && a->act == MMFM_ACT_NONE && !a->D2 && !a->aux && !a->rowdot,
+               "mmfm_gemm_tn_ln: only the fp32 residual epilogue without activation / D2 / aux takes the LayerNorm");
+  MMFM_REQUIRE(a->remap_T == 0 && !a->row_zero, "mmfm_gemm_tn_ln: output-row remap and row_zero are not supported");
+  MMFM_REQUIRE(a->drop.thresh == 0 || a->drop.seed, "mmfm_gemm_tn_ln: dropout without seed pointer");
+  MMFM_REQUIRE(a->drop.thresh < 256, "mmfm_gemm_tn_ln: dropout threshold out of range");
+  MMFM_REQUIRE(al(a->D, 16) && al(a->res, 16) && a->ldd % 4 == 0 && a->ldr % 4 == 0 && a->ldd >= a->N && a->ldr >= a->N,
+               "mmfm_gemm_tn_ln: D / res need 16-byte aligned bases and pitches (multiples of 4 floats, >= N)");
+  MMFM_REQUIRE(ln->gamma && ln->beta,
+               "mmfm_gemm_tn_ln: gamma and beta are required (affine LayerNorm only; ScaleNorm has no fused form)");
+  MMFM_REQUIRE(ln->y && ln->mean && ln->rstd, "mmfm_gemm_tn_ln: null y / mean / rstd");
+  MMFM_REQUIRE(al(ln->gamma, 16) && al(ln->beta, 16) && al(ln->y, 8),
+               "mmfm_gemm_tn_ln: gamma / beta need 16-byte, y 8-byte alignment");
+  MMFM_REQUIRE(ln->modmajor_T <= 0 || (ln->S > 0 && ln->S % ln->modmajor_T == 0 && a->M % ln->S == 0),
+               "mmfm_gemm_tn_ln: modality-major remap needs S %% T == 0 and M %% S == 0");
+  return launch_tn<128, 4, EPI_RES_F32_LN>(a, (cudaStream_t)stream, ln);
+}
+
 static int wgrad_splits(int R, int NO, int KI, int BN, int* rows_per_split) {
   const int tiles = ((NO + kBM - 1) / kBM) * ((KI + BN - 1) / BN);
   const int kblocks = (R + kBK - 1) / kBK;
diff --git a/multi_modal_foundation_model_b200/csrc/norm.cu b/multi_modal_foundation_model_b200/csrc/norm.cu
--- a/multi_modal_foundation_model_b200/csrc/norm.cu
+++ b/multi_modal_foundation_model_b200/csrc/norm.cu
@@ -5,14 +5,6 @@
 namespace mmfm {
 
 constexpr int kLnWarps = 8;
-
-MMFM_DEVINL long long ln_out_row(long long r, int modmajor_T, int S, long long BT) {
-  if (modmajor_T <= 0) return r;
-  const long long b = r / S;
-  const int s = (int)(r - b * S);
-  const int m = s / modmajor_T;
-  return (long long)m * BT + b * modmajor_T + (s - m * modmajor_T);
-}
 
 template <int NV>
 __global__ void __launch_bounds__(kLnWarps * 32) layernorm_fwd_kernel(const float* __restrict__ x,
diff --git a/multi_modal_foundation_model_b200/engine.py b/multi_modal_foundation_model_b200/engine.py
--- a/multi_modal_foundation_model_b200/engine.py
+++ b/multi_modal_foundation_model_b200/engine.py
@@ -455,9 +455,28 @@
                     ops.gemm_tn(A[pre + ".hid"], sh.nat[pre + ".projection"], x0, bias=st.p(pre + ".projection.bias"),
                                 drop=drop, remap=(T, S, off), row_zero=self.zero, res=self.emb[side])
 
-        def attn_block(pre, x_in, x_out, ln_name, mode, nh, p_drop, layer, side, sep):
-            A[ln_name] = b16(R, H)
-            self._ln_fwd(x_in, ln_name, A[ln_name], self.stats)
+        ln_done = set()
+
+        def ln_fwd(x, name, modmajor=False):
+            if name not in ln_done:
+                A[name] = b16(R, H)
+                self._ln_fwd(x, name, A[name], self.stats, modmajor)
+
+        def res_gemm(a, w, x_out, bias, x_in, drop=NO_DROP, next_ln=None, modmajor=False):
+            if not (eng.fuse_ln and next_ln and st.has(next_ln + ".weight") and st.has(next_ln + ".bias")):
+                ops.gemm_tn(a, w, x_out, bias=bias, res=x_in, drop=drop)
+                return
+            A[next_ln] = b16(R, H)
+            mean, rstd = torch.empty(R, device=x_out.device), torch.empty(R, device=x_out.device)
+            self._keep += [mean, rstd]
+            self.stats[next_ln] = (mean, rstd)
+            ops.gemm_tn_ln(a, w, x_out, bias=bias, res=x_in, drop=drop, gamma=st.p(next_ln + ".weight"),
+                           beta=st.p(next_ln + ".bias"), y=A[next_ln], mean=mean, rstd=rstd,
+                           modmajor_T=T if modmajor else 0, S=S if modmajor else 0)
+            ln_done.add(next_ln)
+
+        def attn_block(pre, x_in, x_out, ln_name, mode, nh, p_drop, layer, side, sep, next_ln):
+            ln_fwd(x_in, ln_name)
             A[pre + ".qkv"] = b16(R, 3 * H)
             ops.gemm_tn(A[ln_name], sh.nat[pre + ".qkv"], A[pre + ".qkv"],
                         bias=self._bias([f"{pre}.{k}.bias" for k in ("query", "key", "value")]))
@@ -465,28 +484,26 @@
             A[pre + ".ao"] = b16(R, H)
             self._attention(True, pre, qkv[:, :H], qkv[:, H:2 * H], qkv[:, 2 * H:], A[pre + ".ao"], mode, nh, p_drop,
                             SITE_ATTN_PROB, SITE_ATTN_OUT, layer, side, sep)
-            ops.gemm_tn(A[pre + ".ao"], sh.nat[pre + ".out_proj"], x_out, bias=self._bias([pre + ".out_proj.bias"]),
-                        res=x_in)
-
-        def mlp_block(pre, x_in, x_out, ln_name, p_drop, layer, side, inter):
-            A[ln_name] = b16(R, H)
-            self._ln_fwd(x_in, ln_name, A[ln_name], self.stats)
+            res_gemm(A[pre + ".ao"], sh.nat[pre + ".out_proj"], x_out, self._bias([pre + ".out_proj.bias"]), x_in,
+                     next_ln=next_ln)
+
+        def mlp_block(pre, x_in, x_out, ln_name, p_drop, layer, side, inter, next_ln, modmajor=False):
+            ln_fwd(x_in, ln_name)
             A[pre + ".dg"], A[pre + ".g"] = b16(R, inter), b16(R, inter)
             ops.gemm_tn(A[ln_name], sh.nat[pre + ".up_proj"], A[pre + ".g"], bias=self._bias([pre + ".up_proj.bias"]),
                         act=ACT_GELU_DG if eng.save_gelu_grad else ACT_GELU, D2=A[pre + ".dg"])
-            ops.gemm_tn(A[pre + ".g"], sh.nat[pre + ".down_proj"], x_out, bias=self._bias([pre + ".down_proj.bias"]),
-                        drop=self._drop(SITE_MLP, layer, side, p_drop), res=x_in)
+            res_gemm(A[pre + ".g"], sh.nat[pre + ".down_proj"], x_out, self._bias([pre + ".down_proj.bias"]), x_in,
+                     drop=self._drop(SITE_MLP, layer, side, p_drop), next_ln=next_ln, modmajor=modmajor)
 
         hp = eng.hp
         for i in range(eng.Le):
             pre = f"encoder.{i}"
             self.xs += [f32(R, H), f32(R, H)]
             attn_block(pre + ".attn", self.xs[2 * i], self.xs[2 * i + 1], pre + ".ln1", MASK_KEY_OR_DIAG,
-                       hp["enc_heads"], hp["enc_dropout"], i, SIDE_ENC, False)
+                       hp["enc_heads"], hp["enc_dropout"], i, SIDE_ENC, False, pre + ".ln2")
             mlp_block(pre + ".mlp", self.xs[2 * i + 1], self.xs[2 * i + 2], pre + ".ln2", hp["enc_dropout"], i,
-                      SIDE_ENC, eng.enc_inter)
-        A["encoder_norm"] = b16(R, H)
-        self._ln_fwd(self.xs[-1], "encoder_norm", A["encoder_norm"], self.stats)
+                      SIDE_ENC, eng.enc_inter, f"encoder.{i + 1}.ln1" if i + 1 < eng.Le else "encoder_norm")
+        ln_fwd(self.xs[-1], "encoder_norm")
         self.ctx = f32(R, H)
         ops.gemm_tn(A["encoder_norm"], sh.nat["decoder_proj_context"], self.ctx,
                     bias=st.p("decoder_proj_context.bias"), res=self.emb[SIDE_ENC])
@@ -507,10 +524,9 @@
             self.ys += [f32(R, H), f32(R, H), f32(R, H)]
             y0, y1, y2, y3 = self.ys[3 * i: 3 * i + 4]
             attn_block(pre + ".attn", y0, y1, pre + ".ln1", dec_mode, hp["dec_heads"], hp["dec_dropout"], i, SIDE_DEC,
-                       eng.sep)
+                       eng.sep, pre + ".query_norm")
             xa = pre + ".cross_attn"
-            A[pre + ".query_norm"] = b16(R, H)
-            self._ln_fwd(y1, pre + ".query_norm", A[pre + ".query_norm"], self.stats)
+            ln_fwd(y1, pre + ".query_norm")
             if not eng.fuse_ctx:
                 A[pre + ".context_norm"] = b16(R, H)
                 self._ln_fwd(self.ctx, pre + ".context_norm", A[pre + ".context_norm"], self.stats)
@@ -522,10 +538,12 @@
             self._attention(True, xa, A[xa + ".q"], A[xa + ".kv"][:, :H], A[xa + ".kv"][:, H:], A[xa + ".ao"],
                             MASK_KEY_OR_DIAG, hp["dec_heads"], hp["dec_dropout"], SITE_XATTN_PROB, SITE_XATTN_OUT, i,
                             SIDE_DEC, False)
-            ops.gemm_tn(A[xa + ".ao"], sh.nat[xa + ".out_proj"], y2, bias=self._bias([xa + ".out_proj.bias"]), res=y1)
-            mlp_block(pre + ".mlp", y2, y3, pre + ".ln2", hp["dec_dropout"], i, SIDE_DEC, eng.dec_inter)
-        A["decoder_norm"] = b16(R, H)
-        self._ln_fwd(self.ys[-1], "decoder_norm", A["decoder_norm"], self.stats, modmajor=True)
+            res_gemm(A[xa + ".ao"], sh.nat[xa + ".out_proj"], y2, self._bias([xa + ".out_proj.bias"]), y1,
+                     next_ln=pre + ".ln2")
+            last = i + 1 == eng.Ld
+            mlp_block(pre + ".mlp", y2, y3, pre + ".ln2", hp["dec_dropout"], i, SIDE_DEC, eng.dec_inter,
+                      "decoder_norm" if last else f"decoder.{i + 1}.ln1", modmajor=last)
+        ln_fwd(self.ys[-1], "decoder_norm", modmajor=True)
 
         self.dpreds: Dict[str, torch.Tensor] = {}
         for k, m in enumerate(mods):
@@ -759,6 +777,7 @@
         self.H = model.hidden_size
         self.Le, self.Ld = model.n_enc_layers, model.n_dec_layers
         self.fuse_ctx = fuse_context_norms(dict(model.named_parameters(remove_duplicate=False)), self.Ld)
+        self.fuse_ln = os.environ.get("MMFM_FUSE_LN", "1") != "0" and self.H == 256
         self.causal, self.sep = bool(model.decoder_causal_mask), bool(model.decoder_sep_mask)
         if hp["enc_act"] != "gelu" or hp["dec_act"] != "gelu":
             raise NotImplementedError("only act='gelu' (mm.yaml:44) is built for the transformer MLP")
diff --git a/multi_modal_foundation_model_b200/ops.py b/multi_modal_foundation_model_b200/ops.py
--- a/multi_modal_foundation_model_b200/ops.py
+++ b/multi_modal_foundation_model_b200/ops.py
@@ -133,13 +133,13 @@
     return [(c[2], c[3], evs[i].elapsed_time(evs[i + 1])) for i, c in enumerate(calls)]
 
 
-def gemm_tn(A: torch.Tensor, B: torch.Tensor, D: torch.Tensor, *, M: Optional[int] = None, N: Optional[int] = None,
-            K: Optional[int] = None, bias: Optional[torch.Tensor] = None, res: Optional[torch.Tensor] = None,
-            D2: Optional[torch.Tensor] = None, aux: Optional[torch.Tensor] = None, act: int = ACT_NONE,
-            act_scale: float = 1.0, drop: DropSpec = NO_DROP, remap: Tuple[int, int, int] = (0, 0, 0),
-            row_zero: Optional[torch.Tensor] = None, lda: Optional[int] = None, ldb: Optional[int] = None,
-            ldd: Optional[int] = None, ldr: Optional[int] = None, ldaux: Optional[int] = None,
-            rowdot: Optional[torch.Tensor] = None, rowdot_S: int = 0) -> None:
+def _gemm_args(A: torch.Tensor, B: torch.Tensor, D: torch.Tensor, *, M: Optional[int] = None, N: Optional[int] = None,
+               K: Optional[int] = None, bias: Optional[torch.Tensor] = None, res: Optional[torch.Tensor] = None,
+               D2: Optional[torch.Tensor] = None, aux: Optional[torch.Tensor] = None, act: int = ACT_NONE,
+               act_scale: float = 1.0, drop: DropSpec = NO_DROP, remap: Tuple[int, int, int] = (0, 0, 0),
+               row_zero: Optional[torch.Tensor] = None, lda: Optional[int] = None, ldb: Optional[int] = None,
+               ldd: Optional[int] = None, ldr: Optional[int] = None, ldaux: Optional[int] = None,
+               rowdot: Optional[torch.Tensor] = None, rowdot_S: int = 0) -> Tuple[GemmArgs, float]:
     assert A.dtype == bf16 and B.dtype == bf16 and D.dtype in (bf16, torch.float32)
     a = GemmArgs()
     a.A, a.lda = A.data_ptr(), (lda if lda is not None else A.stride(0))
@@ -167,8 +167,25 @@
     mn = float(a.M) * a.N
     nbytes = 2.0 * a.M * a.K + 2.0 * a.N * a.K + mn * (4 if a.d_fp32 else 2)
     nbytes += (2.0 * mn if D2 is not None else 0.0) + (4.0 * mn if res is not None else 0.0) + (2.0 * mn if aux is not None else 0.0)
+    return a, nbytes
+
+
+def gemm_tn(A: torch.Tensor, B: torch.Tensor, D: torch.Tensor, **kw) -> None:
+    a, nbytes = _gemm_args(A, B, D, **kw)
     _launch("mmfm_gemm_tn", C.byref(a), keep=(a,),
             meta={"flops": 2.0 * a.M * a.N * a.K, "bytes": nbytes, "tag": f"gemm_tn {a.M}x{a.N}x{a.K}"})
+
+
+def gemm_tn_ln(A: torch.Tensor, B: torch.Tensor, D: torch.Tensor, *, res: torch.Tensor, gamma: torch.Tensor,
+               beta: torch.Tensor, y: torch.Tensor, mean: torch.Tensor, rstd: torch.Tensor, eps: float = 1e-5,
+               modmajor_T: int = 0, S: int = 0, **kw) -> None:
+    a, nbytes = _gemm_args(A, B, D, res=res, **kw)
+    assert y.dtype == bf16 and y.stride(0) == a.N and gamma.dtype == beta.dtype == torch.float32
+    ln = _lib.LnEpi(gamma.data_ptr(), beta.data_ptr(), y.data_ptr(), mean.data_ptr(), rstd.data_ptr(), float(eps),
+                    int(modmajor_T), int(S))
+    nbytes += 2.0 * a.M * a.N + 8.0 * a.M
+    _launch("mmfm_gemm_tn_ln", C.byref(a), C.byref(ln), keep=(a, ln),
+            meta={"flops": 2.0 * a.M * a.N * a.K, "bytes": nbytes, "tag": f"gemm_tn_ln {a.M}x{a.N}x{a.K}"})
 
 
 def gemm_wgrad(dY: torch.Tensor, X: torch.Tensor, dW: torch.Tensor, *, R: Optional[int] = None,
```

Measured after the change: 26800 (median of 6 runs). +1.2%, better.
